# mudit1729/dinov2-od

Hardware: AMD Instinct MI355X
Metric: images/sec forward, DINOv2 ViT-B/14 518x518 + 100-query head (higher is better)
Workload: dtype bf16; 1 GPU; ViT-B/14 518x518 bf16, 100 queries, batch 64 per GPU (BASELINE configs[2]'s batch of 64; it fits one GPU, so every GPU runs the whole configuration: weak scaling); global_batch=64, per_gpu_batch=64, image=518, queries=100, parallelism=dp1, hipgraph=True, n_ranks_seen=1, micro_batches=2

## Files before the change

### dinov2_od_amd/_native.py

```python
import ctypes as C
import os

_HERE = os.path.dirname(os.path.abspath(__file__))
LIB_PATH = os.environ.get("DINODET_LIB") or os.path.join(_HERE, "lib", "libdinodet.so")

DOD_F32, DOD_BF16 = 0, 1
PREC = {"fp32": 0, "bf16": 1, "fp8": 2, "bf16x3": 3, "fp16x2": 4}
ACT = {"none": 0, "relu": 1, "gelu": 2, "sigmoid": 3, "swiglu_pairs": 4}
PW = {"gelu_bwd": 0, "swiglu_bwd": 1, "relu_drop_bwd": 2, "dropout_add": 3, "sigmoid_bwd4": 4}


class DodConfig(C.Structure):
    _fields_ = [
        ("hidden", C.c_int32), ("layers", C.c_int32), ("heads", C.c_int32), ("swiglu", C.c_int32),
        ("patch", C.c_int32), ("pos_grid", C.c_int32), ("ffn_hidden", C.c_int32), ("ln_eps", C.c_float),
        ("lora_r", C.c_int32), ("lora_alpha", C.c_float), ("target_dim", C.c_int32),
        ("num_queries", C.c_int32), ("dec_hidden", C.c_int32), ("dec_heads", C.c_int32),
        ("dec_layers", C.c_int32), ("num_classes", C.c_int32), ("dim_feedforward", C.c_int32),
        ("n_points", C.c_int32), ("use_deformable", C.c_int32), ("dec_ln_eps", C.c_float),
        ("precision", C.c_int32),
    ]


_P, _I, _F, _SZ, _I64 = C.c_void_p, C.c_int, C.c_float, C.c_size_t, C.c_int64


class DodDetection(C.Structure):
    _fields_ = [("image_id", C.c_int64), ("category_id", C.c_int32), ("query", C.c_int32), ("bbox", C.c_float * 4),
                ("score", C.c_float), ("reserved", C.c_int32)]

DEC_TRAIN_FIELDS = ["query_embed", "class_w", "class_b", "bb0_w", "bb0_b", "bb2_w", "bb2_b", "in_proj_w", "in_proj_b", "out_proj_w",
                    "out_proj_b", "norm1_w", "norm1_b", "norm2_w", "norm2_b", "norm3_w", "norm3_b", "lin1_w", "lin1_b", "lin2_w", "lin2_b",
                    "refp_w", "refp_b", "off_w", "off_b", "aw_w", "aw_b", "vp_w", "vp_b", "op_w", "op_b"]


class DodDecTrainParams(C.Structure):
    _fields_ = [(f, C.c_void_p) for f in DEC_TRAIN_FIELDS]


DENSE_LAYER_FIELDS = ["sa_in_w", "sa_in_b", "sa_out_w", "sa_out_b", "ca_in_w", "ca_in_b", "ca_out_w", "ca_out_b", "lin1_w", "lin1_b", "lin2_w", "lin2_b",
                      "norm1_w", "norm1_b", "norm2_w", "norm2_b", "norm3_w", "norm3_b"]


class DodDenseLayerParams(C.Structure):
    _fields_ = [(f, C.c_void_p) for f in DENSE_LAYER_FIELDS]


class DodDenseDecTrainParams(C.Structure):
    _fields_ = [("nlayers", C.c_int32), ("reserved", C.c_int32), ("layers", C.POINTER(DodDenseLayerParams))] + \
               [(f, C.c_void_p) for f in ("query_embed", "class_w", "class_b", "bb0_w", "bb0_b", "bb2_w", "bb2_b")]


class DodLoraLinear(C.Structure):
    _fields_ = [("w", C.c_void_p), ("b", C.c_void_p), ("A", C.c_void_p), ("Bm", C.c_void_p)]


class DodBbBlockParams(C.Structure):
    _fields_ = [(f, C.c_void_p) for f in ("ln1_w", "ln1_b", "ln2_w", "ln2_b", "ls1", "ls2")] + \
               [(f, DodLoraLinear) for f in ("q", "k", "v", "o", "fc1", "fc2")]


class DodBbTailParams(C.Structure):
    _fields_ = [("nblocks", C.c_int32), ("reserved", C.c_int32), ("blocks", C.POINTER(DodBbBlockParams)),
                ("lnf_w", C.c_void_p), ("lnf_b", C.c_void_p), ("proj_w", C.c_void_p), ("proj_b", C.c_void_p)]


class DodOptimTensor(C.Structure):
    _fields_ = [("p", C.c_void_p), ("g", C.c_void_p), ("m", C.c_void_p), ("v", C.c_void_p), ("n", C.c_int64),
                ("step_size", C.c_float), ("bc2_sqrt", C.c_float)]


class DodLnFold(C.Structure):
    _fields_ = [("stats", C.c_void_p), ("csum", C.c_void_p), ("op_out", C.c_void_p), ("part", C.c_void_p), ("shift", C.c_void_p),
                ("part_in", C.c_void_p), ("stats_out", C.c_void_p), ("eps", C.c_float)]


class DodDrawLayer(C.Structure):
    _fields_ = [("boxes", C.c_void_p), ("counts", C.c_void_p), ("labels", C.c_void_p), ("scores", C.c_void_p), ("K", C.c_int32),
                ("format", C.c_int32), ("score_threshold", C.c_float), ("use_palette", C.c_int32), ("color", C.c_uint8 * 4)]


class DodDrawStyle(C.Structure):
    _fields_ = [("thickness", C.c_int32), ("fill_alpha", C.c_int32), ("font_scale", C.c_int32), ("palette_size", C.c_int32),
                ("palette", C.c_void_p), ("names", C.c_void_p), ("n_names", C.c_int32), ("name_len", C.c_int32), ("font", C.c_void_p)]


TUNING_SYMBOLS = {
    "dod_debug_gemm_stamps": (_I, [_P]),
    "dod_debug_pp_stamps": (_I, [_P]),
    "dod_debug_attn_stamps": (_I, [_P]),
    "dod_debug_mfma_peak": (_I, [_I, _I, _I, _P, _P]),
    "dod_debug_mfma_valu_probe": (_I, [_I, _I, _I, _I, _P, _P]),
}

SYMBOLS = {
    "dod_create": (_I, [C.POINTER(DodConfig), C.POINTER(_P)]),
    "dod_destroy": (None, [_P]),
    "dod_last_error": (C.c_char_p, [_P]),
    "dod_set_weight": (_I, [_P, C.c_char_p, _P, C.POINTER(C.c_int64), _I, _I]),
    "dod_finalize_weights": (_I, [_P, _P]),
    "dod_prepare": (_I, [_P, _I, _I, _P]),
    "dod_workspace_bytes": (_SZ, [_P, _I, _I, _I]),
    "dod_num_tokens": (_I, [_P, _I, _I]),
    "dod_forward": (_I, [_P, _P, _I, _I, _I, _P, _P, _SZ, _P]),
    "dod_forward_u8": (_I, [_P, _P, _I, _I, _I, _P, _P, _SZ, _P]),
    "dod_backbone_forward": (_I, [_P, _P, _I, _I, _I, _P, _P, _SZ, _P]),
    "dod_backbone_prefix": (_I, [_P, _P, _I, _I, _I, _I, _P, _P, _SZ, _P]),
    "dod_decoder_forward": (_I, [_P, _P, _I, _I, _P, _P, _SZ, _P]),
    "dod_decoder_workspace_bytes": (_SZ, [_P, _I, _I]),
    "dod_set_tap": (_I, [_P, _I, _P]),
    "dod_profile": (_I, [_P, _I]),
    "dod_profile_read": (_I, [_P, _I, C.POINTER(C.c_double), C.POINTER(C.c_double), C.POINTER(C.c_int)]),
    "dod_op_linear": (_I, [_I, _P, _I, _P, _I, _I, _I, _I, _P, _P, _P, _I, _P, _I, _I, _I, _P]),
    "dod_op_gemm_f32x": (_I, [_P, _I, _I, C.c_longlong, C.c_longlong, _P, _I, _I, C.c_longlong, C.c_longlong, _P, _I, C.c_longlong, C.c_longlong,
                         _I, _I, _I, _I, _I, _F, _I, _I, _P]),
    "dod_op_gemm_f32x3": (_I, [_P, _I, _I, C.c_longlong, C.c_longlong, _P, _I, _I, C.c_longlong, C.c_longlong, _P, _I, C.c_longlong, C.c_longlong,
                          _I, _I, _I, _I, _I, _F, _I, _I, _P]),
    "dod_op_linear_f32x3": (_I, [_P, _I, _P, _P, _P, _P, _I, _I, _I, _I, _P, _I, _I, _P]),
    "dod_op_linear_fp8": (_I, [_P, _I, _P, _P, _I, _P, _I, _I, _I, _P, _P, _P, _I, _P, _I, _I, _I, _P]),
    "dod_op_quant_rows_fp8": (_I, [_P, _I, _I, _I, _I, _P, _I, _P, _P]),
    "dod_op_quant_mx_fp8": (_I, [_P, _I, _I, _I, _I, _P, _I, _P, _P]),
    "dod_op_linear_fp8_glu_mx": (_I, [_P, _I, _P, _P, _I, _P, _I, _I, _I, _P, _P, _I, _P, _P]),
    "dod_op_linear_fp8_mx": (_I, [_P, _I, _P, _P, _I, _P, _I, _I, _I, _P, _P, _P, _I, _P, _I, _I, _I, _P]),
    "dod_op_linear_fp8_mx2": (_I, [_P, _I, _P, _P, _I, _P, _I, _I, _I, _P, _P, _P, _I, _P, _I, _I, _I, _P, _P]),
    "dod_op_split_pair": (_I, [_P, _I, _I, _I, _P, _P]),
    "dod_op_linear_x3": (_I, [_P, _P, _I, _I, _I, _P, _P, _P, _I, _P, _I, _I, _I, _P]),
    "dod_op_attention_x3": (_I, [_P, _P, _I, _I, _I, _F, _P]),
    "dod_op_attention_x3_h2": (_I, [_P, _P, _I, _I, _I, _F, _P]),
    "dod_op_split_h2": (_I, [_P, _I, _I, _I, _P, _P, _P]),
    "dod_op_linear_h2": (_I, [_P, _P, _P, _I, _I, _I, _P, _P, _P, _I, _P, _I, _I, _I, _P]),
    "dod_op_layernorm": (_I, [_P, _P, _P, _P, _F, _I, _I, _P, _I, _P]),
    "dod_op_linear_ln": (_I, [_I, _P, _P, _P, _I, _I, _I, _P, _P, _P, _I, _P, _I, _I, _I, C.POINTER(DodLnFold), _P]),
    "dod_op_rowstats": (_I, [_P, _I, _I, _F, _P, _I, _P, _P]),
    "dod_op_ln_finalize": (_I, [_P, _I, _I, _F, _P, _P]),
    "dod_op_attention_bf16": (_I, [_P, _P, _I, _I, _I, _F, _P]),
    "dod_op_attention_bf16_mx": (_I, [_P, _P, _P, _I, _I, _I, _F, _P]),
    "dod_op_attention_f32": (_I, [_P, _P, _P, _P, _I, _I, _I, _I, _I, _I, _I, _I, _I, _F, _P]),
    "dod_op_deform_sample": (_I, [_P, _I, _P, _I, _I, _I, _I, _I, _I, _I, _I, _P, _P]),
    "dod_op_pos_resize": (_I, [_P, _I, _I, _I, _I, _P, _P]),
    "dod_op_im2col": (_I, [_P, _I, _I, _I, _I, _I, _P, _I, _P]),
    "dod_postprocess_workspace_bytes": (_SZ, [_I, _I, _I]),
    "dod_postprocess": (_I, [_P, _I, _I, _I, _P, _F, _P, C.c_int64, _P, _P, _SZ, _P]),
    "dod_detect_workspace_bytes": (_SZ, [_I, _I, _I, _I]),
    "dod_detect": (_I, [_P, _I, _I, _I, _I, _P, _F, _I, _F, _I, _I, _P, _P, _P, _P, _P, _P, _SZ, _P]),
    "dod_detect_views_workspace_bytes": (_SZ, [_I, _I, _I, _I]),
    "dod_detect_views": (_I, [_P, _I, _I, _I, _I, _P, _P, _P, _P, _I, _F, _I, _F, _I, _I, _I, _F, _P, _P, _P, _P, _P, _P, _P, _SZ, _P]),
    "dod_fuse_views_workspace_bytes": (_SZ, [_I, _I, _I, _I]),
    "dod_fuse_views": (_I, [_P, _I, _I, _I, _I, _P, _P, _P, _P, _I, _F, _I, _F, _I, _I, _F, _I, _P, _P, _P, _P, _P, _P, _P, _P, _SZ, _P]),
    "dod_draw_detections": (_I, [_P, _I, _I, _I, _I, C.POINTER(DodDrawLayer), C.POINTER(DodDrawLayer), C.POINTER(DodDrawStyle), _P, _P]),
    "dod_preprocess": (_I, [_P, _P, _P, _P, _I, _I, _I, _I, _I, _P, _P, _P, _P]),
    "dod_preprocess_u8": (_I, [_P, _P, _P, _P, _I, _I, _I, _I, _I, _P, _P, _P, _P]),
    "dod_preprocess_aug": (_I, [_P, _P, _P, _P, _I, _P, _P, _P, _P, _I, _I, _I, _I, _P, _P, _P, _P]),
    "dod_preprocess_aug_u8": (_I, [_P, _P, _P, _P, _I, _P, _P, _P, _P, _I, _I, _I, _I, _P, _P, _P, _P]),
    "dod_preprocess_compose": (_I, [_P, _P, _P, _P, _I, _P, _P, _I, _I, _P, _P, _P, _I, _I, _I, _I, _I, _I, _P, _P, _P, _P]),
    "dod_preprocess_compose_u8": (_I, [_P, _P, _P, _P, _I, _P, _P, _I, _I, _P, _P, _P, _I, _I, _I, _I, _I, _I, _P, _P, _P, _P]),
    "dod_match_cost": (_I, [_P, _I, _I, _I, _P, _P, _P, _I, _F, _F, _F, _F, _F, _I, _P, _P]),
    "dod_match_assign_workspace_bytes": (_SZ, [_I, _I, _I]),
    "dod_match_assign": (_I, [_P, _P, _I, _I, _I, _P, _I, _P, _P, _P, _SZ, _P]),
    "dod_coco_eval_workspace_bytes": (_SZ, [_I64, _I, _I, _I64]),
    "dod_coco_eval_set_gt": (_I, [_P, _SZ, _I64, _I, _I, _I64, _P, _P, _P, _P, _P, _P, _P, _P, _P]),
    "dod_coco_eval_reset": (_I, [_P, _SZ, _I64, _I, _I, _I64, _P]),
    "dod_coco_eval_append": (_I, [_P, _SZ, _I64, _I, _I, _I64, _P, _P, _I64, _P]),
    "dod_coco_eval_append_host": (_I, [_P, _SZ, _I64, _I, _I, _I64, _P, _I64, _P]),
    "dod_coco_eval_evaluate": (_I, [_P, _SZ, _I64, _I, _I, _I64, _P, _P, _P, _P, _P, _P]),
    "dod_coco_eval_matches": (_I, [_P, _SZ, _I64, _I, _I, _I64, _I64, _P, _P, _P, _P, _I, _P, _P, _P]),
    "dod_op_sort_pairs_workspace_bytes": (_SZ, [_I64]),
    "dod_op_sort_pairs_u64": (_I, [_P, _P, _P, _P, _I64, _I, _I, _P, _SZ, _P]),
    "dod_set_criterion_workspace_bytes": (_SZ, [_I, _I, _I]),
    "dod_set_criterion_forward": (_I, [_P, C.c_int64, _P, C.c_int64, _I, _I, _I, _P, _P, _I, _P, _I, _P, _F, _F, _P, _P, _P, _SZ, _P]),
    "dod_set_criterion_backward": (_I, [_P, C.c_int64, _P, C.c_int64, _I, _I, _I, _P, _P, _I, _P, _I, _P, _F, _F, _P, _P, _P, _P, _P]),
    "dod_set_criterion_layers_workspace_bytes": (_SZ, [_I, _I, _I, _I]),
    "dod_set_criterion_layers_forward": (_I, [_P, C.c_int64, _P, C.c_int64, _I, _I, _I, _I, _P, _P, _I, _P, _I, _P, _F, _F, _P, _P, _P, _SZ, _P]),
    "dod_set_criterion_layers_backward": (_I, [_P, C.c_int64, _P, C.c_int64, _I, _I, _I, _I, _P, _P, _I, _P, _I, _P, _F, _F, _P, _P, _P, _P, _P]),
    "dod_decoder_train_aux_tape_bytes": (_SZ, [C.POINTER(DodConfig), _I, _I]),
    "dod_decoder_train_aux_workspace_bytes": (_SZ, [C.POINTER(DodConfig), _I, _I]),
    "dod_decoder_train_aux_forward": (_I, [C.POINTER(DodConfig), _P, _P, _I, _I, _F, C.c_uint64, _P, _P, _SZ, _P, _SZ, _P]),
    "dod_decoder_train_aux_backward": (_I, [C.POINTER(DodConfig), _P, _P, _I, _I, _F, C.c_uint64, _P, _P, _SZ, _P, _P, _P, _SZ, _P]),
    "dod_decoder_train_tape_bytes": (_SZ, [C.POINTER(DodConfig), _I, _I]),
    "dod_decoder_train_workspace_bytes": (_SZ, [C.POINTER(DodConfig), _I, _I]),
    "dod_decoder_train_forward": (_I, [C.POINTER(DodConfig), _P, _P, _I, _I, _F, C.c_uint64, _P, _P, _SZ, _P, _SZ, _P]),
    "dod_decoder_train_backward": (_I, [C.POINTER(DodConfig), _P, _P, _I, _I, _F, C.c_uint64, _P, _P, _SZ, _P, _P, _P, _SZ, _P]),
    "dod_decoder_train_last_error": (C.c_char_p, []),
    "dod_dense_decoder_train_tape_bytes": (_SZ, [C.POINTER(DodConfig), _I, _I]),
    "dod_dense_decoder_train_workspace_bytes": (_SZ, [C.POINTER(DodConfig), _I, _I]),
    "dod_dense_decoder_train_forward": (_I, [C.POINTER(DodConfig), _P, _P, _I, _I, _F, C.c_uint64, _P, _P, _SZ, _P, _SZ, _P]),
    "dod_dense_decoder_train_backward": (_I, [C.POINTER(DodConfig), _P, _P, _I, _I, _F, C.c_uint64, _P, _P, _SZ, _P, _P, _P, _SZ, _P]),
    "dod_backbone_tail_tape_bytes": (_SZ, [C.POINTER(DodConfig), _I, _I, _I]),
    "dod_backbone_tail_workspace_bytes": (_SZ, [C.POINTER(DodConfig), _I, _I, _I]),
    "dod_backbone_tail_train_forward": (_I, [C.POINTER(DodConfig), _P, _P, _I, _I, _P, _P, _SZ, _P, _SZ, _P]),
    "dod_backbone_tail_train_backward": (_I, [C.POINTER(DodConfig), _P, _I, _I, _P, _P, _SZ, _P, _P, _SZ, _P]),
    "dod_op_layernorm_bwd": (_I, [_P, _P, _P, _F, _I, _I, _P, _P, _P, _P]),
    "dod_op_attention_f32_vjp_workspace_bytes": (_SZ, [_I, _I, _I, _I, _I, _I]),
    "dod_op_attention_f32_vjp": (_I, [_P, _I, _P, _P, _I, _P, _P, _I, _P, _I, _P, _P, _I, _I, _I, _I, _I, _I, _F, _I, _F, C.c_uint64, _P, _SZ, _P]),
    "dod_op_deform_sample_bwd": (_I, [_P, _I, _P, _P, _I, _I, _I, _I, _I, _I, _I, _I, _P, _P, _P]),
    "dod_op_lora_grads_workspace_bytes": (_SZ, [_I, _I]),
    "dod_op_lora_grads": (_I, [_P, _I, _P, _I, _I, _P, _P, _I, _I, _F, _P, _P, _P, _SZ, _P]),
    "dod_op_train_pointwise": (_I, [_I, _P, _P, _P, _SZ, _I, _F, C.c_uint64, _P]),
    "dod_op_colsum_add": (_I, [_P, _I, _I, _I, _P, _P]),
    "dod_optim_workspace_bytes": (_SZ, [_I, _I64]),
    "dod_optim_clip_grad_norm": (_I, [_P, _I, _F, _P, _P, _SZ, _P]),
    "dod_optim_adam_step": (_I, [_P, _I, C.c_double, C.c_double, _F, C.c_double, _F, _P, _P, _SZ, _P]),
    "dod_optim_last_error": (C.c_char_p, []),
    "dod_reserve_gemm_scratch": (_I, [C.c_size_t]),
    "dod_test_set_option": (_I, [C.c_char_p, _I]),
    "dod_test_counter": (C.c_long, [C.c_char_p]),
    "dod_test_gemm_plan": (_I, [_I, _I, _I, _I, C.c_uint, _I, C.c_size_t, _P, _I]),
    "dod_version": (C.c_char_p, []),
    "dod_abi_version": (_I, []),
    "dod_device_count": (_I, []),
}

_lib = None
ABI_VERSION = 6


def lib():
    global _lib
    if _lib is None:
        import torch
        if not os.path.exists(LIB_PATH):
            raise RuntimeError(
                f"{LIB_PATH} not found: the HIP extension is required (no CPU fallback). "
                "Build it with `python -m dinov2_od_amd._build`.")
        L = C.CDLL(LIB_PATH)
        other = bool(os.environ.get("DINODET_LIB"))
        for name, (res, args) in SYMBOLS.items():
            if other and not hasattr(L, name):
                continue
            fn = getattr(L, name)
            fn.restype = res
            fn.argtypes = args
        for name, (res, args) in TUNING_SYMBOLS.items():
            if hasattr(L, name):
                fn = getattr(L, name)
                fn.restype = res
                fn.argtypes = args
        if L.dod_abi_version() != ABI_VERSION and not other:
            raise RuntimeError(f"{LIB_PATH} has ABI revision {L.dod_abi_version()}, this binding expects {ABI_VERSION}: rebuild it "
                               "(`python -m dinov2_od_amd._build --force`)")
        try:
            if torch.cuda.is_available() and L.dod_device_count() <= 0:
                raise RuntimeError("libdinodet.so is bound to a different HIP runtime than PyTorch "
                                   "(it sees no device): import torch before loading it")
        except AttributeError:
            pass
        _lib = L
    return _lib


class DodGemmStep(C.Structure):
    _fields_ = [(n, C.c_int) for n in ("form", "row0", "rows", "kslices", "regmath", "gm")]


def gemm_plan(family, M, N, K, epi_flags, cus, scratch_bytes):
    steps = (DodGemmStep * 4)()
    n = lib().dod_test_gemm_plan(family, M, N, K, epi_flags, cus, scratch_bytes, steps, 4)
    if n < 0:
# ... 30 lines not shown
```

### dinov2_od_amd/csrc/dod_api.hip

```cpp
#include "dod_internal.h"
#include "gemm_plan.h"

#include <cstdarg>
#include <cstdio>
#include <atomic>
#include <cstdlib>

using namespace dod;

static std::string g_err;

static int vfail(const dod_handle* h, int code, const char* fmt, va_list ap, int launch_rc = 0) {
  char buf[512];
  const int n = vsnprintf(buf, sizeof buf, fmt, ap);
  if (launch_rc && n >= 0 && (size_t)n < sizeof buf) snprintf(buf + n, sizeof buf - n, " rejected (rc %d)", launch_rc);
  if (h) h->err = buf; else g_err = buf;
  return code;
}
int dod::fail(const dod_handle* h, int code, const char* fmt, ...) {
  va_list ap; va_start(ap, fmt); code = vfail(h, code, fmt, ap); va_end(ap);
  return code;
}
int dod::rejected(const dod_handle* h, int r, const char* fmt, ...) {
  if (!r) return DOD_OK;
  va_list ap; va_start(ap, fmt); const int code = vfail(h, r == 3 ? DOD_ERR_HIP : DOD_ERR_INVALID, fmt, ap, r); va_end(ap);
  return code;
}

static bool check_common(dod_handle* h, int B, int H, int W, int* rc) {
  if (!h) { *rc = fail(nullptr, DOD_ERR_INVALID, "null handle"); return false; }
  if (!h->finalized) { *rc = fail(h, DOD_ERR_STATE, "dod_finalize_weights has not been called"); return false; }
  if (B <= 0) { *rc = fail(h, DOD_ERR_INVALID, "batch must be positive (got %d)", B); return false; }
  if (H < h->cfg.patch || W < h->cfg.patch) { *rc = fail(h, DOD_ERR_INVALID, "image %dx%d smaller than one %dx%d patch", H, W, h->cfg.patch, h->cfg.patch); return false; }
  return true;
}

static std::atomic<int> g_options[DOD_OPT_COUNT] = {{-1}, {-1}, {-1}, {-1}, {-1}, {-1}, {-1}, {-1}, {-1}, {-1}, {-1}};
int dod_option(int which) { return which >= 0 && which < DOD_OPT_COUNT ? g_options[which].load() : -1; }
static const char* const k_option_names[DOD_OPT_COUNT] = {"tailsplit", "dec_fused_split", "mha_chunk_images", "no_fused_patch", "ln_fold", "deterministic", "f32_ksplit",
                                                       "attn_bwd_flash", "epi_regmath", "f32x3_tile", "attn_diet"};

static std::atomic<long> g_form_launches[FORM_COUNT];
static const char* const k_form_names[FORM_COUNT] = {"bf16_128_r2", "bf16_128_r3", "bf16_m16", "k64", "ppm", "x3_16w", "x3_pp", "h2", "fp8_rows", "fp8mx_256x128",
                                                     "fp8mx2_256x128", "fp8mx2_256x256", "f32", "patch_fused"};
void gemm_form_launched(int form) { if (form >= 0 && form < FORM_COUNT) ++g_form_launches[form]; }

extern "C" {

int dod_test_set_option(const char* name, int value) {
  if (!name) return fail(nullptr, DOD_ERR_INVALID, "null option name");
  for (int i = 0; i < DOD_OPT_COUNT; ++i)
    if (!strcmp(name, k_option_names[i])) { g_options[i].store(value); return DOD_OK; }
  return fail(nullptr, DOD_ERR_INVALID, "unknown test option '%s'", name);
}
long dod_test_counter(const char* name) {
  if (name && !strcmp(name, "tail_splits")) return gemm_tail_split_count();
  if (name && !strcmp(name, "rem_cuts")) return gemm_rem_cut_count();
  if (name && !strcmp(name, "f32_ksplits")) return gemm_f32_ksplit_count();
  if (name && !strcmp(name, "epi_regmath")) return gemm_epi_regmath_count();
  if (name && !strcmp(name, "attn_diet")) return attn_half_tile_count();
  if (name && !strcmp(name, "f32x3_launches")) return gemm_f32x3_count(0);
  if (name && !strcmp(name, "f32x3_wide_launches")) return gemm_f32x3_count(1);
  if (name && !strcmp(name, "optim_launches")) return optim_launch_count();
  if (name && !strcmp(name, "optim_chunk_elems")) return optim_constant(0);
  if (name && !strcmp(name, "optim_table_tensors")) return optim_constant(1);
  if (name && !strcmp(name, "optim_norm_table_tensors")) return optim_constant(2);
  if (name && !strncmp(name, "form_", 5))
    for (int i = 0; i < FORM_COUNT; ++i)
      if (!strcmp(name + 5, k_form_names[i])) return g_form_launches[i].load();
  return -1;
}

int dod_test_gemm_plan(int family, int M, int N, int K, unsigned epi_flags, int cus, size_t scratch_bytes, dod_gemm_step* steps, int max_steps) {
  if (family < GEMM_BF16 || family > GEMM_F32 || M <= 0 || N <= 0 || K <= 0 || cus <= 0 || !steps) return -1;
  const GemmPlan pl = gemm_plan(family, M, N, K, epi_flags, gemm_policy(cus, scratch_bytes, scratch_bytes > 0));
  if (pl.n > 4 || pl.n > max_steps) return -1;
  for (int i = 0; i < pl.n; ++i) {
    const GemmStep& st = pl.step[i];
    steps[i].form = st.form; steps[i].row0 = st.row0; steps[i].rows = st.rows; steps[i].kslices = st.kslices; steps[i].regmath = st.regmath; steps[i].gm = st.gm;
  }
  return pl.n;
}

const char* dod_version(void) { return "dinodet 0.3 (gfx950)"; }
int dod_abi_version(void) { return DOD_ABI_VERSION; }

int dod_device_count(void) {
  int n = 0;
  return hipGetDeviceCount(&n) == hipSuccess ? n : -1;
}

const char* dod_last_error(const dod_handle* h) { return h ? h->err.c_str() : g_err.c_str(); }

int dod_create(const dod_config* cfg, dod_handle** out) {
  if (!cfg || !out) return fail(nullptr, DOD_ERR_INVALID, "null argument");
  const dod_config& c = *cfg;
  if (c.hidden <= 0 || c.layers <= 0 || c.heads <= 0 || c.hidden % c.heads) return fail(nullptr, DOD_ERR_INVALID, "bad backbone dims hidden=%d heads=%d layers=%d", c.hidden, c.heads, c.layers);
  if (c.hidden % 64) return fail(nullptr, DOD_ERR_INVALID, "hidden (%d) must be a multiple of 64", c.hidden);
  {
    const int fm = c.precision == DOD_PREC_FP32 ? 4 : 64;
    if (c.ffn_hidden <= 0 || c.ffn_hidden % fm) return fail(nullptr, DOD_ERR_INVALID, "ffn_hidden (%d) must be a multiple of %d in this precision", c.ffn_hidden, fm);
  }
  if (c.patch <= 0 || c.pos_grid <= 0) return fail(nullptr, DOD_ERR_INVALID, "bad patch/pos_grid");
  if (c.num_queries <= 0 || c.dec_hidden <= 0 || c.dec_heads <= 0 || c.dec_layers <= 0 || c.num_classes <= 0 || c.dim_feedforward <= 0) return fail(nullptr, DOD_ERR_INVALID, "bad decoder dims");
  if (c.dec_hidden % 64 || c.dim_feedforward % 4) return fail(nullptr, DOD_ERR_INVALID, "decoder hidden (%d) must be a multiple of 64, dim_feedforward (%d) of 4", c.dec_hidden, c.dim_feedforward);
  if (c.target_dim && c.target_dim != c.dec_hidden) return fail(nullptr, DOD_ERR_INVALID, "projection dim %d != decoder hidden %d", c.target_dim, c.dec_hidden);
  if (!c.target_dim && c.hidden != c.dec_hidden) return fail(nullptr, DOD_ERR_INVALID, "backbone width %d != decoder hidden %d and no projection", c.hidden, c.dec_hidden);
  if (c.use_deformable && (c.n_points <= 0 || c.n_points > 8)) return fail(nullptr, DOD_ERR_INVALID, "n_points must be 1..8");
  if (c.dec_layers > 64) return fail(nullptr, DOD_ERR_INVALID, "at most 64 decoder layers");
  if (c.precision != DOD_PREC_FP32 && c.precision != DOD_PREC_BF16 && c.precision != DOD_PREC_FP8 && c.precision != DOD_PREC_BF16X3 && c.precision != DOD_PREC_FP16X2) return fail(nullptr, DOD_ERR_INVALID, "unknown precision %d", c.precision);
  dod_handle* h = new (std::nothrow) dod_handle();
  if (!h) return fail(nullptr, DOD_ERR_STATE, "out of host memory");
  h->cfg = c;
  *out = h;
  return DOD_OK;
}

void dod_destroy(dod_handle* h) {
  if (!h) return;
  for (auto& r : h->prof) { (void)hipEventDestroy(r.a); (void)hipEventDestroy(r.b); }
  for (auto e : h->evpool) (void)hipEventDestroy(e);
  for (void* p : h->owned) (void)hipFree(p);
  delete h;
}

int dod_set_weight(dod_handle* h, const char* key, const void* dev_ptr, const int64_t* shape, int ndim, int dtype) {
  if (!h || !key || !dev_ptr || ndim < 0 || ndim > 8 || (ndim && !shape)) return fail(h, DOD_ERR_INVALID, "dod_set_weight: bad argument");
  if (dtype != DOD_F32 && dtype != DOD_BF16) return fail(h, DOD_ERR_INVALID, "dod_set_weight('%s'): dtype %d is neither DOD_F32 nor DOD_BF16", key, dtype);
  std::string k(key);
  if (k.rfind("module.", 0) == 0) k = k.substr(7);
  WRef r; r.raw = dev_ptr; r.dtype = dtype; r.ptr = dtype == DOD_F32 ? (const float*)dev_ptr : nullptr; r.shape.assign(shape, shape + ndim);
  h->w[k] = r;
  h->finalized = false;
  return DOD_OK;
}

int dod_reserve_gemm_scratch(size_t bytes) { return (gemm_tail_reserve(bytes) || gemm_f32_ksplit_reserve()) ? fail(nullptr, DOD_ERR_HIP, "scratch allocation of %zu bytes failed", bytes) : DOD_OK; }

int dod_finalize_weights(dod_handle* h, void* stream) {
  if (!h) return fail(nullptr, DOD_ERR_INVALID, "null handle");
  { static const size_t mb = [] { const char* v = getenv("DINODET_GEMM_SCRATCH_MB"); return v && atoi(v) > 0 ? (size_t)atoi(v) : (size_t)64; }();
    (void)gemm_tail_reserve(mb << 20);
    (void)gemm_f32_ksplit_reserve(); }
  int rc = finalize_impl(h, (hipStream_t)stream);
  if (rc || !h->has_dec) return rc;
  hipStream_t s = (hipStream_t)stream;
  const dod_config& g = h->cfg;
  const size_t Q = g.num_queries, Dd = g.dec_hidden;
  h->l0_tgt = h->l0_proj = nullptr;
  Carver sz(nullptr);
  const size_t bytes = carve_decoder(h, sz, 1, 1, nullptr, false) + 256;
  void* tmp = nullptr;
  float *t0 = nullptr, *p0 = nullptr;
  HIPCHK(h, hipMalloc(&tmp, bytes));
  if (hipMalloc((void**)&t0, Q * Dd * 4) != hipSuccess || (g.use_deformable && hipMalloc((void**)&p0, Q * (size_t)h->ncat * 4) != hipSuccess)) {
    (void)hipFree(tmp); if (t0) (void)hipFree(t0);
    return fail(h, DOD_ERR_HIP, "allocation of the decoder's layer-0 constants failed");
  }
  h->owned.push_back(t0); if (p0) h->owned.push_back(p0);
  Carver cv((void*)(((uintptr_t)tmp + 255) & ~(uintptr_t)255));
  DecWS dw;
  carve_decoder(h, cv, 1, 1, &dw, false);
  rc = decoder_impl(h, nullptr, 1, 1, dw, nullptr, s, true);
  if (!rc) {
    hipError_t e1 = hipMemcpyAsync(t0, dw.tgt, Q * Dd * 4, hipMemcpyDeviceToDevice, s);
    hipError_t e2 = p0 ? hipMemcpyAsync(p0, dw.proj, Q * (size_t)h->ncat * 4, hipMemcpyDeviceToDevice, s) : hipSuccess;
    hipError_t e3 = hipStreamSynchronize(s);
    if (e1 != hipSuccess || e2 != hipSuccess || e3 != hipSuccess) rc = fail(h, DOD_ERR_HIP, "decoder layer-0 constants: %s", hipGetErrorString(e3 != hipSuccess ? e3 : (e1 != hipSuccess ? e1 : e2)));
  } else (void)hipStreamSynchronize(s);
  (void)hipFree(tmp);
  if (rc) return rc;
  h->l0_tgt = t0; h->l0_proj = p0;
  return DOD_OK;
}

int dod_prepare(dod_handle* h, int H, int W, void* stream) {
  if (!h) return fail(nullptr, DOD_ERR_INVALID, "null handle");
  return prepare_impl(h, H, W, (hipStream_t)stream);
}

int dod_num_tokens(const dod_handle* h, int H, int W) { return h ? (H / h->cfg.patch) * (W / h->cfg.patch) + 1 : 0; }

size_t dod_workspace_bytes(const dod_handle* h, int B, int H, int W) {
  if (!h || B <= 0 || H < h->cfg.patch || W < h->cfg.patch) return 0;
  const int N = dod_num_tokens(h, H, W);
  Carver c(nullptr);
  carve_backbone(h, c, B, N, nullptr);
  carve_decoder(h, c, B, N, nullptr, false);
  return c.off + 256;
}

size_t dod_decoder_workspace_bytes(const dod_handle* h, int B, int N) {
  if (!h || B <= 0 || N <= 0) return 0;
  Carver c(nullptr);
  carve_decoder(h, c, B, N, nullptr, true);
  return c.off + 256;
}

int dod_set_tap(dod_handle* h, int stage, float* dst) {
  if (!h) return fail(nullptr, DOD_ERR_INVALID, "null handle");
  if (dst) h->taps[stage] = dst; else h->taps.erase(stage);
  return DOD_OK;
}

int dod_forward(dod_handle* h, const float* pixels, int B, int H, int W, float* det, void* workspace, size_t wsb, void* stream) {
  int rc;
  if (!check_common(h, B, H, W, &rc)) return rc;
  if (!pixels || !det || !workspace) return fail(h, DOD_ERR_INVALID, "null buffer");
  if (wsb < dod_workspace_bytes(h, B, H, W)) return fail(h, DOD_ERR_STATE, "workspace too small: %zu < %zu", wsb, dod_workspace_bytes(h, B, H, W));
  const int N = dod_num_tokens(h, H, W);
  Carver c(align_ws(workspace));
  BbWS bw; DecWS dw;
  carve_backbone(h, c, B, N, &bw);
  carve_decoder(h, c, B, N, &dw, false);
  CARVE_FITS(h, c, workspace, wsb)
  rc = backbone_impl(h, pixels, B, H, W, bw, nullptr, true, (hipStream_t)stream); if (rc) return rc;
  return decoder_impl(h, bw.mem, B, N, dw, det, (hipStream_t)stream);
}

int dod_forward_u8(dod_handle* h, const uint8_t* pixels_hwc, int B, int H, int W, float* det, void* workspace, size_t wsb, void* stream) {
  int rc;
  if (!check_common(h, B, H, W, &rc)) return rc;
  if (!pixels_hwc || !det || !workspace) return fail(h, DOD_ERR_INVALID, "null buffer");
  if (wsb < dod_workspace_bytes(h, B, H, W)) return fail(h, DOD_ERR_STATE, "workspace too small: %zu < %zu", wsb, dod_workspace_bytes(h, B, H, W));
  const int N = dod_num_tokens(h, H, W);
  Carver c(align_ws(workspace));
  BbWS bw; DecWS dw;
  carve_backbone(h, c, B, N, &bw);
  carve_decoder(h, c, B, N, &dw, false);
  CARVE_FITS(h, c, workspace, wsb)
  rc = backbone_impl(h, nullptr, B, H, W, bw, nullptr, true, (hipStream_t)stream, -1, nullptr, pixels_hwc); if (rc) return rc;
  return decoder_impl(h, bw.mem, B, N, dw, det, (hipStream_t)stream);
}

int dod_backbone_forward(dod_handle* h, const float* pixels, int B, int H, int W, float* features, void* workspace, size_t wsb, void* stream) {
  int rc;
  if (!check_common(h, B, H, W, &rc)) return rc;
  if (!pixels || !features || !workspace) return fail(h, DOD_ERR_INVALID, "null buffer");
  if (wsb < dod_workspace_bytes(h, B, H, W)) return fail(h, DOD_ERR_STATE, "workspace too small: %zu < %zu", wsb, dod_workspace_bytes(h, B, H, W));
  const int N = dod_num_tokens(h, H, W);
  Carver c(align_ws(workspace));
  BbWS bw;
  carve_backbone(h, c, B, N, &bw);
  CARVE_FITS(h, c, workspace, wsb)
  return backbone_impl(h, pixels, B, H, W, bw, features, false, (hipStream_t)stream);
}

int dod_backbone_prefix(dod_handle* h, const float* pixels, int B, int H, int W, int nblocks, float* x_out, void* workspace, size_t wsb, void* stream) {
  int rc;
  if (!check_common(h, B, H, W, &rc)) return rc;
  if (!pixels || !x_out || !workspace) return fail(h, DOD_ERR_INVALID, "null buffer");
  if (nblocks < 0 || nblocks > h->cfg.layers) return fail(h, DOD_ERR_INVALID, "nblocks %d outside 0..%d", nblocks, h->cfg.layers);
  if (wsb < dod_workspace_bytes(h, B, H, W)) return fail(h, DOD_ERR_STATE, "workspace too small: %zu < %zu", wsb, dod_workspace_bytes(h, B, H, W));
  const int N = dod_num_tokens(h, H, W);
  Carver c(align_ws(workspace));
  BbWS bw;
  carve_backbone(h, c, B, N, &bw);
  CARVE_FITS(h, c, workspace, wsb)
  return backbone_impl(h, pixels, B, H, W, bw, nullptr, false, (hipStream_t)stream, nblocks, x_out);
}

int dod_decoder_forward(dod_handle* h, const float* memory, int B, int N, float* det, void* workspace, size_t wsb, void* stream) {
  if (!h) return fail(nullptr, DOD_ERR_INVALID, "null handle");
  if (!h->finalized) return fail(h, DOD_ERR_STATE, "dod_finalize_weights has not been called");
  if (B <= 0 || N <= 0) return fail(h, DOD_ERR_INVALID, "bad B=%d N=%d", B, N);
  if (!memory || !det || !workspace) return fail(h, DOD_ERR_INVALID, "null buffer");
  if (wsb < dod_decoder_workspace_bytes(h, B, N)) return fail(h, DOD_ERR_STATE, "workspace too small");
  Carver c(align_ws(workspace));
  DecWS dw;
  carve_decoder(h, c, B, N, &dw, true);
  CARVE_FITS(h, c, workspace, wsb)
  hipStream_t s = (hipStream_t)stream;
  const void* mem_op = memory;
  if (is_bf16(h)) {
    KCHK(h, launch_cast_bf16(memory, (bf16_t*)dw.mem_op, (size_t)B * N * h->cfg.dec_hidden, s));
    mem_op = dw.mem_op;
  }
  return decoder_impl(h, mem_op, B, N, dw, det, s);
}

int dod_profile(dod_handle* h, int enable) {
  if (!h) return fail(nullptr, DOD_ERR_INVALID, "null handle");
  for (auto& r : h->prof) { h->evpool.push_back(r.a); h->evpool.push_back(r.b); }
  h->prof.clear();
  h->prof_on = enable != 0;
  return DOD_OK;
}

int dod_profile_read(dod_handle* h, int cls, double* ms, double* flops, int* launches) {
  if (!h || cls < 0 || cls >= PC_COUNT) return fail(h, DOD_ERR_INVALID, "bad profile class");
  double t = 0, f = 0; int n = 0;
  for (auto& r : h->prof) {
    if (r.cls != cls) continue;
    HIPCHK(h, hipEventSynchronize(r.b));
    float e = 0.f;
    HIPCHK(h, hipEventElapsedTime(&e, r.a, r.b));
    t += e; f += r.flops; ++n;
  }
  if (ms) *ms = t; if (flops) *flops = f; if (launches) *launches = n;
  return DOD_OK;
}

int dod_op_linear(int in_dtype, const void* A, int lda, const void* W, int ldw, int M, int N, int K, const float* bias,
                  const float* scale, const float* resid, int ldr, void* out, int out_dtype, int ldc, int act, void* stream) {
  if (!A || !W || !out) return fail(nullptr, DOD_ERR_INVALID, "null buffer");
  GemmEpi e = epi(bias, out_dtype == DOD_F32 ? (float*)out : nullptr, out_dtype == DOD_BF16 ? out : nullptr, ldc, act, scale, resid, ldr);
  if (act == DOD_ACT_SWIGLU_PAIRS) {
    if (in_dtype != DOD_BF16 || out_dtype != DOD_BF16 || scale || resid || (N & 7)) return fail(nullptr, DOD_ERR_INVALID, "DOD_ACT_SWIGLU_PAIRS: bf16 in / out, N %% 8 == 0, no scale / residual");
    e.act = ACT_NONE; e.glu = 1;
  }
  int r = in_dtype == DOD_BF16 ? launch_gemm_bf16((const bf16_t*)A, lda, (const bf16_t*)W, ldw, M, N, K, e, (hipStream_t)stream)
                               : launch_gemm_f32((const float*)A, lda, (const float*)W, ldw, M, N, K, e, (hipStream_t)stream);
  return rejected(nullptr, r, "dod_op_linear M=%d N=%d K=%d", M, N, K);
}
int dod_op_gemm_f32x(const float* A, int lda, int a_kmajor, long long a_sb, long long a_sh, const float* W, int ldw, int w_kmajor, long long w_sb,
                     long long w_sh, float* C, int ldc, long long c_sb, long long c_sh, int M, int N, int K, int batch, int hb, float alpha,
                     int accumulate, int ksplit, void* stream) {
  if (!A || !W || !C) return fail(nullptr, DOD_ERR_INVALID, "null buffer");
  GemmF32X g; memset(&g, 0, sizeof g);
  g.A = A; g.lda = lda; g.a_kmajor = a_kmajor; g.a_sb = a_sb; g.a_sh = a_sh;
  g.W = W; g.ldw = ldw; g.w_kmajor = w_kmajor; g.w_sb = w_sb; g.w_sh = w_sh;
  g.C = C; g.ldc = ldc; g.c_sb = c_sb; g.c_sh = c_sh;
  g.M = M; g.N = N; g.K = K; g.batch = batch; g.hb = hb; g.alpha = alpha; g.accumulate = accumulate; g.ksplit = ksplit;
  return rejected(nullptr, launch_gemm_f32x(g, (hipStream_t)stream), "dod_op_gemm_f32x M=%d N=%d K=%d batch=%d", M, N, K, batch);
}
int dod_op_gemm_f32x3(const float* A, int lda, int a_kmajor, long long a_sb, long long a_sh, const float* W, int ldw, int w_kmajor, long long w_sb,
                      long long w_sh, float* C, int ldc, long long c_sb, long long c_sh, int M, int N, int K, int batch, int hb, float alpha,
                      int accumulate, int ksplit, void* stream) {
  if (!A || !W || !C) return fail(nullptr, DOD_ERR_INVALID, "null buffer");
  GemmF32X g; memset(&g, 0, sizeof g);
  g.A = A; g.lda = lda; g.a_kmajor = a_kmajor; g.a_sb = a_sb; g.a_sh = a_sh;
  g.W = W; g.ldw = ldw; g.w_kmajor = w_kmajor; g.w_sb = w_sb; g.w_sh = w_sh;
  g.C = C; g.ldc = ldc; g.c_sb = c_sb; g.c_sh = c_sh;
  g.M = M; g.N = N; g.K = K; g.batch = batch; g.hb = hb; g.alpha = alpha; g.accumulate = accumulate; g.ksplit = ksplit;
  return rejected(nullptr, launch_gemm_f32x3(g, (hipStream_t)stream), "dod_op_gemm_f32x3 M=%d N=%d K=%d batch=%d", M, N, K, batch);
}
int dod_op_linear_f32x3(const float* X, int ldx, const float* W, const float* bias, const float* scale, const float* resid, int ldr, int M, int N, int K,
                        float* Y, int ldy, int act, void* stream) {
  if (!X || !W || !Y) return fail(nullptr, DOD_ERR_INVALID, "null buffer");
  if (act < DOD_ACT_NONE || act > DOD_ACT_SIGMOID) return fail(nullptr, DOD_ERR_INVALID, "dod_op_linear_f32x3: activation %d", act);
  GemmF32X g; memset(&g, 0, sizeof g);
  g.A = X; g.lda = ldx; g.W = W; g.ldw = K; g.C = Y; g.ldc = ldy; g.M = M; g.N = N; g.K = K; g.batch = 1; g.hb = 1; g.alpha = 1.0f; g.ksplit = 1;
  g.bias = bias; g.scale = scale; g.resid = resid; g.ldr = ldr; g.act = act;
  return rejected(nullptr, launch_gemm_f32x3(g, (hipStream_t)stream), "dod_op_linear_f32x3 M=%d N=%d K=%d", M, N, K);
}
int dod_op_linear_fp8(const void* A, int lda, const float* a_scale, const void* W, int ldw, const float* w_scale, int M, int N, int K,
                      const float* bias, const float* scale, const float* resid, int ldr, void* out, int out_dtype, int ldc, int act,
                      void* stream) {
  if (!A || !W || !out || !a_scale || !w_scale) return fail(nullptr, DOD_ERR_INVALID, "null buffer");
  GemmEpi e = epi(bias, out_dtype == DOD_F32 ? (float*)out : nullptr, out_dtype == DOD_BF16 ? out : nullptr, ldc, act, scale, resid, ldr);
  e.a_scale = a_scale; e.w_scale = w_scale;
  return rejected(nullptr, launch_gemm_fp8((const unsigned char*)A, lda, (const unsigned char*)W, ldw, M, N, K, e, (hipStream_t)stream), "dod_op_linear_fp8 M=%d N=%d K=%d", M, N, K);
}
int dod_op_linear_fp8_mx(const void* A, int lda, const void* a_block_scales, const void* W, int ldw, const float* w_scale, int M, int N, int K,
                         const float* bias, const float* scale, const float* resid, int ldr, void* out, int out_dtype, int ldc, int act,
                         void* stream) {
  if (!A || !W || !out || !a_block_scales || !w_scale) return fail(nullptr, DOD_ERR_INVALID, "null buffer");
  GemmEpi e = epi(bias, out_dtype == DOD_F32 ? (float*)out : nullptr, out_dtype == DOD_BF16 ? out : nullptr, ldc, act, scale, resid, ldr);
  e.a_bs = (const unsigned char*)a_block_scales; e.w_scale = w_scale;
  return rejected(nullptr, launch_gemm_fp8((const unsigned char*)A, lda, (const unsigned char*)W, ldw, M, N, K, e, (hipStream_t)stream), "dod_op_linear_fp8_mx M=%d N=%d K=%d", M, N, K);
}
int dod_op_linear_fp8_glu_mx(const void* A, int lda, const float* a_scale, const void* W, int ldw, const float* w_scale, int M, int N, int K,
                             const float* bias, void* out_q, int ldq, void* out_block_scales, void* stream) {
  if (!A || !W || !a_scale || !w_scale || !out_q || !out_block_scales) return fail(nullptr, DOD_ERR_INVALID, "null buffer");
  GemmEpi e = epi(bias, nullptr, out_q, ldq);
  e.a_scale = a_scale; e.w_scale = w_scale; e.glu = 1; e.out_bs = (unsigned char*)out_block_scales;
  return rejected(nullptr, launch_gemm_fp8((const unsigned char*)A, lda, (const unsigned char*)W, ldw, M, N, K, e, (hipStream_t)stream), "dod_op_linear_fp8_glu_mx M=%d N=%d K=%d", M, N, K);
}
int dod_op_linear_fp8_mx2(const void* A, int lda, const void* a_block_scales, const void* W, int ldw, const void* w_block_scales, int M, int N, int K,
                          const float* bias, const float* scale, const float* resid, int ldr, void* out, int out_dtype, int ldc, int act,
                          void* glu_out_block_scales, void* stream) {
  if (!A || !W || !out || !a_block_scales || !w_block_scales) return fail(nullptr, DOD_ERR_INVALID, "null buffer");
// ... 125 lines not shown
```

### dinov2_od_amd/csrc/dod_common.h

```cpp
#pragma once
#include <hip/hip_runtime.h>
#include <stdint.h>
#include <stdlib.h>

typedef __attribute__((ext_vector_type(8))) __bf16 bf16x8;
typedef __attribute__((ext_vector_type(4))) __bf16 bf16x4;
typedef __attribute__((ext_vector_type(2))) __bf16 bf16x2;
typedef __attribute__((ext_vector_type(16))) float f32x16;
typedef __attribute__((ext_vector_type(4))) float f32x4;
typedef __attribute__((ext_vector_type(2))) float f32x2;
typedef unsigned short bf16_t;

#define DOD_WAVE 64

enum { DOD_OPT_TAILSPLIT = 0,
       DOD_OPT_DEC_FUSED_SPLIT,
       DOD_OPT_MHA_CHUNK_IMAGES,
       DOD_OPT_NO_FUSED_PATCH,
       DOD_OPT_LN_FOLD,
       DOD_OPT_DETERMINISTIC,
       DOD_OPT_F32_KSPLIT,
       DOD_OPT_ATTN_BWD_FLASH,
       DOD_OPT_EPI_REGMATH,
       DOD_OPT_F32X3_TILE,
       DOD_OPT_ATTN_DIET,
       DOD_OPT_COUNT };
int dod_option(int which);
long gemm_tail_split_count();
long optim_launch_count();
long optim_constant(int which);
long gemm_rem_cut_count();
long attn_half_tile_count();
long gemm_epi_regmath_count();
enum { FORM_BF16_128_R2 = 0, FORM_BF16_128_R3, FORM_BF16_M16, FORM_K64, FORM_PPM, FORM_X3_16W, FORM_X3_PP, FORM_H2, FORM_FP8_ROWS, FORM_FP8MX_256X128,
       FORM_FP8MX2_256X128, FORM_FP8MX2_256X256, FORM_F32, FORM_PATCH_FUSED, FORM_COUNT };
void gemm_form_launched(int form);
enum { GEMM_BF16 = 0, GEMM_X3, GEMM_H2, GEMM_FP8, GEMM_F32 };

#ifdef DINODET_TUNING
#define DOD_TUNE_ENV(name) getenv(name)
#else
#define DOD_TUNE_ENV(name) (static_cast<const char*>(nullptr))
#endif

__device__ __forceinline__ bf16_t f2bf(float f) {
  __bf16 b = (__bf16)f;
  return __builtin_bit_cast(bf16_t, b);
}
__device__ __forceinline__ float bf2f(bf16_t h) {
  return __builtin_bit_cast(float, ((uint32_t)h) << 16);
}
__device__ __forceinline__ uint32_t pack2bf(float lo, float hi) {
  f32x2 v = {lo, hi};
  bf16x2 h = __builtin_convertvector(v, bf16x2);
  return __builtin_bit_cast(uint32_t, h);
}
__device__ __forceinline__ float wave_sum(float v) {
#pragma unroll
  for (int o = 32; o > 0; o >>= 1) v += __shfl_xor(v, o, 64);
  return v;
}
__device__ __forceinline__ float wave_max(float v) {
#pragma unroll
  for (int o = 32; o > 0; o >>= 1) v = fmaxf(v, __shfl_xor(v, o, 64));
  return v;
}
__device__ __forceinline__ unsigned pack4_fp8(float a, float b, float c, float d) {
  int w = __builtin_amdgcn_cvt_pk_fp8_f32(a, b, 0, false);
  w = __builtin_amdgcn_cvt_pk_fp8_f32(c, d, w, true);
  return (unsigned)w;
}
__device__ __forceinline__ unsigned mx_ebyte(float amax) {
  const unsigned b = __float_as_uint(amax * (1.0f / 448.0f));
  unsigned eb = ((b >> 23) & 0xffu) + ((b & 0x7fffffu) ? 1u : 0u);
  eb = eb < 1u ? 1u : (eb > 253u ? 253u : eb);
  return eb;
}
__device__ __forceinline__ float mx_inv_scale(unsigned eb) { return __uint_as_float((254u - eb) << 23); }
__device__ __forceinline__ size_t mx_scale_off(int K, int bi) { return (size_t)(bi & 1) * (K >> 6) + (bi >> 1); }
typedef __attribute__((ext_vector_type(2))) _Float16 f16x2;
typedef __attribute__((ext_vector_type(8))) _Float16 f16x8;
__device__ __forceinline__ float clampf_(float v, float lim) { return __builtin_fminf(__builtin_fmaxf(v, -lim), lim); }
__device__ __forceinline__ void h2_quad(float4 v, float shi, uint2& f16, unsigned& hi8, unsigned& lo8) {
  v.x = clampf_(v.x, 65504.f); v.y = clampf_(v.y, 65504.f); v.z = clampf_(v.z, 65504.f); v.w = clampf_(v.w, 65504.f);
  const f16x2 p0 = {(_Float16)v.x, (_Float16)v.y}, p1 = {(_Float16)v.z, (_Float16)v.w};
  f16.x = __builtin_bit_cast(unsigned, p0); f16.y = __builtin_bit_cast(unsigned, p1);
  const float hx = (float)p0.x, hy = (float)p0.y, hz = (float)p1.x, hw = (float)p1.y;
  const float slo = shi * 2048.0f;
  hi8 = pack4_fp8(clampf_(hx * shi, 448.f), clampf_(hy * shi, 448.f), clampf_(hz * shi, 448.f), clampf_(hw * shi, 448.f));
  lo8 = pack4_fp8(clampf_((v.x - hx) * slo, 448.f), clampf_((v.y - hy) * slo, 448.f), clampf_((v.z - hz) * slo, 448.f), clampf_((v.w - hw) * slo, 448.f));
}
__device__ __forceinline__ size_t h2_off8(int K, int c) { return (size_t)2 * K + (size_t)(c >> 4) * 32 + (c & 15); }

__device__ __forceinline__ float gelu_erf(float x) { return 0.5f * x * (1.0f + erff(x * 0.70710678118654752440f)); }
typedef float f32x2_t __attribute__((ext_vector_type(2)));
__device__ __forceinline__ f32x2_t gelu_fast2(f32x2_t x) {
  f32x2_t ax; ax.x = __builtin_fabsf(x.x); ax.y = __builtin_fabsf(x.y);
  const f32x2_t z = ax * 0.8493218002880191f;
  const f32x2_t d = __builtin_elementwise_fma(z, (f32x2_t)(0.2727374808792225f), (f32x2_t)(1.0f));
  f32x2_t t; t.x = __builtin_amdgcn_rcpf(d.x); t.y = __builtin_amdgcn_rcpf(d.y);
  f32x2_t p = __builtin_elementwise_fma(t, (f32x2_t)(0.5f * 1.061405429f), (f32x2_t)(0.5f * -1.453152027f));
  p = __builtin_elementwise_fma(p, t, (f32x2_t)(0.5f * 1.421413741f));
  p = __builtin_elementwise_fma(p, t, (f32x2_t)(0.5f * -0.284496736f));
  p = __builtin_elementwise_fma(p, t, (f32x2_t)(0.5f * 0.254829592f));
  const f32x2_t nz2 = -z * z;
  f32x2_t e; e.x = __builtin_amdgcn_exp2f(nz2.x); e.y = __builtin_amdgcn_exp2f(nz2.y);
  const f32x2_t q = ax * (t * p);
  const f32x2_t r = __builtin_elementwise_fma(ax, (f32x2_t)(0.5f), x * 0.5f);
  return __builtin_elementwise_fma(-q, e, r);
}
__device__ __forceinline__ void gelu_fast4(float4& v) {
  f32x2_t a = {v.x, v.y}, b = {v.z, v.w};
  a = gelu_fast2(a); b = gelu_fast2(b);
  v.x = a.x; v.y = a.y; v.z = b.x; v.w = b.y;
}
__device__ __forceinline__ float sigmoidf_(float x) { return 1.0f / (1.0f + expf(-x)); }

enum { ACT_NONE = 0, ACT_RELU = 1, ACT_GELU = 2, ACT_SIGMOID = 3 };

struct GemmEpi {
  const float* bias;
  const float* scale;
  const float* resid;
  int ldr;
  float* out_f32;
  bf16_t* out_bf16;
  int ldc;
  int act;
  const float* pos;
  int rows_per_img;
  int out_rows_per_img;
  int out_split;
  const float* a_scale;
  const float* w_scale;
  unsigned char* out_bs;
  const unsigned char* a_bs;
  const unsigned char* w_bs;
  int out_h2;
  const unsigned char* h2_wexp;
  int ksplit;
  int kslice_len;
  long long kslice_stride;
  int glu;
  void* ln_op;
  int ln_op_kind;
  int ln_op_ld;
  float2* ln_part;
  int ln_npart;
  const float2* ln_shift;
  const float2* ln_stats;
  const float* ln_c;
  const float2* ln_part_in;
  float2* ln_stats_out;
  float ln_eps;
};
enum { LNOP_BF16 = 1, LNOP_PAIR = 2, LNOP_H2 = 3 };
inline bool gemm_epi_rows_ok(const GemmEpi& e) {
  return e.rows_per_img == 0 && !e.pos && e.ksplit <= 1 && !e.a_scale && !e.a_bs && !e.out_bs;
}
inline GemmEpi gemm_epi_rows(const GemmEpi& e, int m0) {
  GemmEpi r = e;
  const size_t m = (size_t)m0;
  if (r.resid) r.resid += m * r.ldr;
  if (r.out_f32) r.out_f32 += m * r.ldc;
  if (r.out_bf16) r.out_bf16 += m * r.ldc;
  if (r.ln_op) r.ln_op = reinterpret_cast<char*>(r.ln_op) + m * (size_t)r.ln_op_ld * 2;
  if (r.ln_part) r.ln_part += m * r.ln_npart;
  if (r.ln_shift) r.ln_shift += m;
  if (r.ln_stats) r.ln_stats += m;
  if (r.ln_part_in) r.ln_part_in += m * r.ln_npart;
  if (r.ln_stats_out) r.ln_stats_out += m;
  return r;
}

int launch_gemm_bf16(const bf16_t* A, int lda, const bf16_t* W, int ldw, int M, int N, int K,
                     const GemmEpi& e, hipStream_t s);
int launch_gemm_f32(const float* A, int lda, const float* W, int ldw, int M, int N, int K,
                    const GemmEpi& e, hipStream_t s, bool allow_ksplit = false);
int gemm_f32_ksplit_reserve();
long gemm_f32_ksplit_count();
struct GemmF32X {
  const float* A; const float* W; float* C; const float* bias;
  const float* scale;
  const float* resid;
  int ldr;
  int lda, ldw, ldc, M, N, K;
  long long a_sb, a_sh, w_sb, w_sh, c_sb, c_sh;
  int batch, hb;
  int a_kmajor, w_kmajor;
  float alpha;
  int accumulate;
  int act;
  int ksplit;
};
int launch_gemm_f32x(const GemmF32X& g, hipStream_t s);
int launch_gemm_f32x3(const GemmF32X& g, hipStream_t s);
long gemm_f32x3_count(int wide);
int launch_quant_mx_fp8(const void* x, int in_bf16, int ld, int rows, int cols, unsigned char* q, int ldq, unsigned char* bs, hipStream_t s);
int launch_gemm_fp8(const unsigned char* A, int lda, const unsigned char* W, int ldw, int M, int N, int K,
                    const GemmEpi& e, hipStream_t s);
int launch_attn_x3(const bf16_t* qkv2, bf16_t* ctx3, int B, int N, int heads, float scale, hipStream_t s, int ctx_h2 = 0);
int launch_swiglu_fp8(const bf16_t* in, int rows, int Fh, unsigned char* q, float* scale, hipStream_t s);
int launch_quant_rows_fp8(const void* x, int in_bf16, int ld, int rows, int cols, unsigned char* q, int ldq, float* scale,
                          hipStream_t s);

struct LnOut {
  float* f32 = nullptr;
  bf16_t* bf16 = nullptr;
  unsigned char* fp8 = nullptr;
  float* scale = nullptr;
  bf16_t* split = nullptr;
  bf16_t* a3 = nullptr;
  unsigned char* bs = nullptr;
};
inline LnOut ln_out(float* f32, bf16_t* bf16 = nullptr, bf16_t* a3 = nullptr) { LnOut o; o.f32 = f32; o.bf16 = bf16; o.a3 = a3; return o; }
int launch_layernorm(const float* x, const float* add, const float* gamma, const float* beta, float eps, int rows, int D, const LnOut& out,
                     hipStream_t s, int split_h2 = 0);
int launch_rowstats(const float* x, int rows, int D, float eps, void* op, int op_kind, float2* stats, hipStream_t s);
int launch_ln_finalize(const float2* part, int npart, int rows, int D, float eps, float2* stats, hipStream_t s);
int launch_ln_fold(const float* W, int rows, int cols, const float* gamma, const float* beta, const float* bias_in, float* Wout, float* bias_out, hipStream_t s);
int launch_rowsum(const float* W, int rows, int cols, int round_bf16, float* c, hipStream_t s);

int launch_attn_bf16(const bf16_t* qkv, bf16_t* ctx, int B, int N, int heads, float scale, hipStream_t s, unsigned char* ctx_bs = nullptr);

struct AttnF32 {
  const float *q, *k, *v; float* o;
  int ldq, ldk, ldv, ldo;
  int Lq, Lk;
  int B, heads, dh;
  float scale;
  bf16_t* o3 = nullptr;
  float* lse = nullptr;
};
int launch_attn_f32(const AttnF32& a, hipStream_t s);
struct AttnF32Bwd {
  const float *q, *k, *v, *o, *d_o, *lse;
  float *dq, *dk, *dv, *delta;
  int ldq, ldk, ldv, ldo, lddq, lddk, lddv;
  int Lq, Lk, B, heads, dh;
  float scale;
};
int launch_attn_f32_bwd(const AttnF32Bwd& a, hipStream_t s);

int launch_im2col(const float* img, int B, int H, int W, int patch, int Kp, float* out_f32, bf16_t* out_bf16, hipStream_t s);
int launch_patch_pack(const float* W, int D, int p, bf16_t* out, int x3, hipStream_t s);
int launch_patch_embed(const void* img, int u8, int B, int H, int W, int p, const bf16_t* Wp, int x3, const float* bias, const float* pos,
                       float* out, int D, hipStream_t s);
int launch_cls_row(const float* cls, const float* pos, float* x, int B, int N, int D, hipStream_t s);
int launch_pos_resize(const float* pos_in, int G, int gh, int gw, int D, float* pos_out, hipStream_t s);
int launch_interleave_halves(const float* src, float* dst, int F, int cols, hipStream_t s);
int launch_swiglu(const float* in_f32, const bf16_t* in_bf16, int rows, int Fh, float* out_f32, bf16_t* out_bf16, hipStream_t s);
int launch_cast_bf16(const float* in, bf16_t* out, size_t n, hipStream_t s);
int launch_copy2d(const float* src, int ld_src, float* dst, int ld_dst, int rows, int cols, int cols_pad, hipStream_t s);
int launch_lora_merge(const float* W, const float* A, const float* Bm, float alpha, int out_f, int in_f, int r, float* dst, hipStream_t s);
int launch_split3(const float* in, int ld_in, bf16_t* out, int rows, int K, int mode, hipStream_t s);
int launch_split2(const float* in, int ld_in, bf16_t* out, int rows, int K, hipStream_t s);
int launch_split_h2(const float* in, int ld_in, void* out, int rows, int K, unsigned char* wexp, hipStream_t s);
int launch_gemm_h2(const void* A, int lda, const void* W, int ldw, int M, int N, int K, const GemmEpi& e, hipStream_t s);
int launch_gemm_x3(const bf16_t* A2, int lda, const bf16_t* W2, int ldw, int M, int N, int K, const GemmEpi& e, hipStream_t s);
int gemm_dispatch(int family, const void* A, int lda, const void* W, int ldw, int M, int N, int K, const GemmEpi& e, hipStream_t s, bool allow_ksplit = false);
int device_cus();
struct KernelLds { const void* fn; int bytes; };
void gemm_lds_attr_once(bool* done, const KernelLds* k, int n);
int gemm_tile_mode();
int run_gemm_bf16_128(const bf16_t* A, int lda, const bf16_t* W, int ldw, int M, int N, int K, const GemmEpi& e, int slots, hipStream_t s);
int run_gemm_bf16_m16(const bf16_t* A, int lda, const bf16_t* W, int ldw, int M, int N, int K, const GemmEpi& e, int gm, hipStream_t s);
int run_gemm_x3_16w(const bf16_t* A2, int lda, const bf16_t* W2, int ldw, int M, int N, int K, const GemmEpi& e, hipStream_t s);
int run_gemm_k64(const bf16_t* A, int lda, const bf16_t* W, int ldw, int M, int N, int K, const GemmEpi& e, bool regmath, hipStream_t s);
int run_gemm_pp(bool x3, const bf16_t* A, int lda, const bf16_t* W, int ldw, int M, int N, int K, const GemmEpi& e, hipStream_t s);
int run_gemm_h2(const void* A, int lda, const void* W, int ldw, int M, int N, int K, const GemmEpi& e, hipStream_t s);
int run_gemm_ksplit_reduce(const float* part, int S, int R, int N, const GemmEpi& e, int m_base, int M, int K, hipStream_t s);
int run_gemm_fp8(int form, const unsigned char* A, int lda, const unsigned char* W, int ldw, int M, int N, int K, const GemmEpi& e, int gm, hipStream_t s);
int run_gemm_f32(const float* A, int lda, const float* W, int ldw, int M, int N, int K, const GemmEpi& e, int S, hipStream_t s);
int gemm_tail_reserve(size_t bytes);
size_t gemm_tail_reserved();
float* gemm_tail_slab(hipStream_t s);
bool gemm_f32_ksplit_reserved();
int launch_bcast_rows(const float* src, float* dst, int B, int rows, int D, hipStream_t s);

int launch_deform_sample(const float* proj, int ldp, const float* values, int B, int Q, int N, int Hd, int P, int dh,
                         int h, int w, float* out, hipStream_t s, int proj_shared = 0, bf16_t* out3 = nullptr);
```

### dinov2_od_amd/csrc/dod_forward.hip

```cpp
#include "dod_internal.h"

#include <cmath>
#include <cstdlib>

using namespace dod;

size_t dod::carve_decoder(const dod_handle* h, Carver& c, int B, int N, DecWS* w, bool need_mem_op) {
  const dod_config& g = h->cfg;
  const size_t BQ = (size_t)B * g.num_queries, Dd = g.dec_hidden, M = (size_t)B * N;
  DecWS t;
  t.tgt = (float*)c.take(BQ * Dd * 4); t.t2 = (float*)c.take(BQ * Dd * 4); t.att = (float*)c.take(BQ * Dd * 4);
  t.samp = (float*)c.take(BQ * Dd * 4); t.qkv = (float*)c.take(BQ * 3 * Dd * 4);
  t.proj = (float*)c.take(BQ * (size_t)(h->ncat > 0 ? h->ncat : 4) * 4);
  t.ffn = (float*)c.take(BQ * (size_t)g.dim_feedforward * 4); t.hb = (float*)c.take(BQ * (Dd / 2) * 4);
  t.qd = (float*)c.take(BQ * Dd * 4);
  { const size_t kmax = Dd > (size_t)g.dim_feedforward ? Dd : (size_t)g.dim_feedforward;
    const bool want3 = is_bf16(h) || is_x3(h);
    t.a3 = want3 ? (bf16_t*)c.take(BQ * 3 * kmax * 2) : nullptr;
    t.a3b = want3 ? (bf16_t*)c.take(BQ * 3 * kmax * 2) : nullptr; }
  t.mem2 = is_x3(h) ? (bf16_t*)c.take(M * 2 * Dd * 2) : nullptr;
  t.mem_op = need_mem_op ? c.take(M * Dd * esz(h)) : nullptr;
  if (g.use_deformable) {
    int uniq = 0; for (auto& L : h->DL) if (L.vp_alias < 0) ++uniq;
    if (!h->finalized) uniq = g.dec_layers;
    t.values = (float*)c.take(M * Dd * 4 * (size_t)(uniq > 0 ? uniq : 1)); t.kv = nullptr;
  } else {
    t.values = nullptr; t.kv = (float*)c.take(M * 2 * Dd * 4);
  }
  if (w) *w = t;
  return c.off;
}

size_t dod::carve_backbone(const dod_handle* h, Carver& c, int B, int N, BbWS* w) {
  const dod_config& g = h->cfg;
  const size_t M = (size_t)B * N, D = g.hidden, es = esz(h), Np = N - 1;
  const size_t F1 = g.swiglu ? 2 * (size_t)g.ffn_hidden : (size_t)g.ffn_hidden;
  size_t hb = M * F1; const size_t col = (size_t)B * Np * (size_t)(h->Kp ? h->Kp : (3 * g.patch * g.patch + 63) / 64 * 64);
  if (col > hb) hb = col;
  BbWS t;
  t.x = (float*)c.take(M * D * 4); t.y = c.take(M * D * es); t.qkv = c.take(M * 3 * D * es); t.ctx = c.take(M * D * es);
  t.hbuf = c.take(hb * es); t.gated = g.swiglu ? c.take(M * (size_t)g.ffn_hidden * es) : nullptr;
  t.mem = c.take(M * (size_t)(g.target_dim ? g.target_dim : g.hidden) * es);
  t.rs = is_fp8(h) ? (float*)c.take(M * 4) : nullptr;
  t.bs = (is_fp8(h) && g.swiglu && g.ffn_hidden % 256 == 0) ? (unsigned char*)c.take(M * (size_t)(g.ffn_hidden / 32)) : nullptr;
  t.bsx = (is_fp8(h) && D % 256 == 0) ? (unsigned char*)c.take(M * (D / 32)) : nullptr;
  const bool foldable = ln_foldable(h);
  t.lnp = foldable ? (float2*)c.take(M * ((D + 127) / 128) * 8) : nullptr;
  t.lns = foldable ? (float2*)c.take(M * 8) : nullptr;
  t.lns2 = foldable ? (float2*)c.take(M * 8) : nullptr;
  if (w) *w = t;
  return c.off;
}

int dod::prepare_impl(dod_handle* h, int H, int W, hipStream_t s) {
  const dod_config& g = h->cfg;
  if (!h->finalized || !h->has_bb) return fail(h, DOD_ERR_STATE, "backbone weights not finalized");
  if (H < g.patch || W < g.patch) return fail(h, DOD_ERR_INVALID, "image %dx%d smaller than one patch", H, W);
  if (h->pos_H == H && h->pos_W == W) return DOD_OK;
  const int gh = H / g.patch, gw = W / g.patch;
  if (gh * gw == g.pos_grid * g.pos_grid && H == W) { h->pos_hw = h->pos; h->pos_H = H; h->pos_W = W; return DOD_OK; }
  const std::pair<int, int> key(gh, gw);
  auto it = h->pos_cache.find(key);
  if (it == h->pos_cache.end()) {
    hipStreamCaptureStatus cs = hipStreamCaptureStatusNone;
    if (s && hipStreamIsCapturing(s, &cs) == hipSuccess && cs != hipStreamCaptureStatusNone)
      return fail(h, DOD_ERR_STATE, "first forward at %dx%d inside a stream capture: call dod_prepare(h, %d, %d) before capturing", H, W, H, W);
    const size_t need = (size_t)(gh * gw + 1) * g.hidden;
    float* buf = nullptr;
    HIPCHK(h, hipMalloc((void**)&buf, need * 4));
    h->owned.push_back(buf);
    KCHK(h, launch_pos_resize(h->pos, g.pos_grid, gh, gw, g.hidden, buf, s));
    it = h->pos_cache.emplace(key, buf).first;
  }
  h->pos_hw = it->second; h->pos_H = H; h->pos_W = W;
  return DOD_OK;
}

namespace {

void spatial_factor(int hw, int* h, int* w) {
  int s = (int)std::sqrt((double)hw);
  while ((s + 1) * (s + 1) <= hw) ++s;
  while (s * s > hw) --s;
  if (s * s != hw) {
    for (int i = s; i > 0; --i) if (hw % i == 0) { *h = i; *w = hw / i; return; }
  }
  *h = s; *w = s;
}

int tap(dod_handle* h, int stage, const void* src, bool src_bf16, size_t n, hipStream_t s) {
  auto it = h->taps.find(stage);
  if (it == h->taps.end() || !it->second) return 0;
  if (!src_bf16) { (void)hipMemcpyAsync(it->second, src, n * 4, hipMemcpyDeviceToDevice, s); return 0; }
  return launch_widen_bf16((const bf16_t*)src, it->second, n, s);
}

int linear(dod_handle* h, bool bf, const void* A, int lda, const void* W, int ldw, int M, int N, int K, const GemmEpi& e, hipStream_t s, int flops_K = 0) {
  ProfScope ps(h, s, bf ? PC_GEMM_BF16 : PC_GEMM_F32, 2.0 * M * N * (e.rows_per_img > 0 ? 3.0 * h->cfg.patch * h->cfg.patch : (double)(flops_K ? flops_K : K)));
  int r = bf ? launch_gemm_bf16((const bf16_t*)A, lda, (const bf16_t*)W, ldw, M, N, K, e, s)
             : launch_gemm_f32((const float*)A, lda, (const float*)W, ldw, M, N, K, e, s, h->cfg.precision != DOD_PREC_FP32);
  return rejected(h, r, "linear launch (M=%d N=%d K=%d bf16=%d)", M, N, K, (int)bf);
}
int linear3(dod_handle* h, const void* A3, const void* W3, int M, int N, int K, const GemmEpi& e, hipStream_t s) {
  ProfScope ps(h, s, PC_GEMM_BF16, 2.0 * M * N * (double)K);
  int r = launch_gemm_x3((const bf16_t*)A3, 2 * K, (const bf16_t*)W3, 2 * K, M, N, K, e, s);
  return rejected(h, r, "bf16x3 linear launch (M=%d N=%d K=%d)", M, N, K);
}

struct Operand {
  const void* rows;
  const float* row_scale = nullptr;
  const unsigned char* bs = nullptr;
};

int block_linear(dod_handle* h, const Operand& a, const PackedLinear& W, int M, int N, int K, GemmEpi e, hipStream_t s) {
  if (is_h2(h)) {
    ProfScope ps(h, s, PC_GEMM_BF16, 2.0 * M * N * (double)K);
    e.h2_wexp = W.wexp;
    return rejected(h, launch_gemm_h2(a.rows, 4 * K, W.W, 3 * K, M, N, K, e, s), "fp16x2 linear launch (M=%d N=%d K=%d)", M, N, K);
  }
  if (is_x3(h)) return linear3(h, a.rows, W.W, M, N, K, e, s);
  if (W.wscale || W.wbs) {
    ProfScope ps(h, s, PC_GEMM_FP8, 2.0 * M * N * (double)K);
    e.a_scale = a.row_scale; e.w_scale = W.wscale; e.a_bs = a.bs; e.w_bs = W.wbs;
    return rejected(h, launch_gemm_fp8((const unsigned char*)a.rows, K, (const unsigned char*)W.W, K, M, N, K, e, s), "fp8 linear launch (M=%d N=%d K=%d)", M, N, K);
  }
  return linear(h, is_bf16(h), a.rows, K, W.W, K, M, N, K, e, s);
}

struct BlockRun {
  dod_handle* h; const BbWS& ws; hipStream_t s;
  int B, N, M, D, F;
  bool bf, f8, x3, h2, fold;
  float scale;
  float2* stat[2];
  int cur = 0;
  bool fresh = false;
  int op_kind, npart;

  BlockRun(dod_handle* h_, const BbWS& ws_, hipStream_t s_, int B_, int N_, bool fold_)
      : h(h_), ws(ws_), s(s_), B(B_), N(N_), M(B_ * N_), D(h_->cfg.hidden), F(h_->cfg.ffn_hidden), bf(is_bf16(h_)), f8(is_fp8(h_)), x3(is_x3(h_)),
        h2(is_h2(h_)), fold(fold_), scale(1.0f / std::sqrt((float)(h_->cfg.hidden / h_->cfg.heads))), stat{ws_.lns, ws_.lns2},
        op_kind(is_h2(h_) ? LNOP_H2 : (is_x3(h_) ? LNOP_PAIR : LNOP_BF16)), npart((h_->cfg.hidden + 127) / 128) {}

  bool mx(const BLayer& L) const { return f8 && L.qkv.wbs && ws.bsx; }

  GemmEpi residual_epi(const PackedLinear& W, const float* layer_scale, bool next_norm_reads) {
    GemmEpi e = epi(W.bias, ws.x, nullptr, D, ACT_NONE, layer_scale, ws.x, D);
    if (fold && next_norm_reads) {
      e.ln_op = ws.y; e.ln_op_kind = op_kind; e.ln_op_ld = (op_kind == LNOP_BF16 ? D : 2 * D); e.ln_part = ws.lnp; e.ln_npart = npart; e.ln_shift = stat[cur];
      fresh = true;
    }
    return e;
  }
  GemmEpi normed_epi(GemmEpi e, const PackedLinear& W) {
    if (fold) {
      e.ln_stats = stat[cur]; e.ln_c = W.csum;
      if (fresh) { e.ln_part_in = ws.lnp; e.ln_npart = npart; e.ln_stats_out = stat[cur ^ 1]; e.ln_eps = h->cfg.ln_eps; cur ^= 1; fresh = false; }
    }
    return e;
  }
  int norm(const BLayer& L, const float* gamma, const float* beta, Operand* y) {
    *y = Operand{ws.y, f8 && !mx(L) ? ws.rs : nullptr, mx(L) ? ws.bsx : nullptr};
    if (fold) return 0;
    LnOut o;
    if (x3) o.split = (bf16_t*)ws.y;
    else if (f8) { o.fp8 = (unsigned char*)ws.y; o.scale = (float*)y->row_scale; o.bs = (unsigned char*)y->bs; }
    else if (bf) o.bf16 = (bf16_t*)ws.y;
    else o.f32 = (float*)ws.y;
    ProfScope ps(h, s, PC_LAYERNORM, 0);
    KCHK(h, launch_layernorm(ws.x, nullptr, gamma, beta, h->cfg.ln_eps, M, D, o, s, h2 ? 1 : 0));
    return 0;
  }
  int attention(const BLayer& L, const Operand& y, Operand* ctx) {
    const int heads = h->cfg.heads;
    const bool flash = D / heads == 64;
    GemmEpi eq = epi(L.qkv.bias, bf ? nullptr : (float*)ws.qkv, bf ? ws.qkv : nullptr, 3 * D);
    if (x3 && flash) { eq = epi(L.qkv.bias, nullptr, ws.qkv, 6 * D); eq.out_split = -3 * D; }
    int rc = block_linear(h, y, L.qkv, M, 3 * D, D, normed_epi(eq, L.qkv), s); if (rc) return rc;
    const double flops = 4.0 * B * (double)N * N * D;
    *ctx = Operand{ws.ctx};
    if (x3 && flash) {
      ProfScope ps(h, s, PC_ATTN_BF16, flops);
      KCHK(h, launch_attn_x3((const bf16_t*)ws.qkv, (bf16_t*)ws.ctx, B, N, heads, scale, s, h2 ? 1 : 0));
    } else if (bf && mx(L)) {
      ProfScope ps(h, s, PC_ATTN_BF16, flops);
      KCHK(h, launch_attn_bf16((const bf16_t*)ws.qkv, (bf16_t*)ws.y, B, N, heads, scale, s, ws.bsx));
      *ctx = Operand{ws.y, nullptr, ws.bsx};
    } else if (bf) {
      { ProfScope ps(h, s, PC_ATTN_BF16, flops); KCHK(h, launch_attn_bf16((const bf16_t*)ws.qkv, (bf16_t*)ws.ctx, B, N, heads, scale, s)); }
      if (f8) {
        KCHK(h, launch_quant_rows_fp8(ws.ctx, 1, D, M, D, (unsigned char*)ws.y, D, ws.rs, s));
        *ctx = Operand{ws.y, ws.rs};
      }
    } else {
      float* o = x3 ? (float*)ws.hbuf : (float*)ws.ctx;
      {
        ProfScope ps(h, s, PC_ATTN_F32, flops);
        AttnF32 a; const float* q = (const float*)ws.qkv;
        a.q = q; a.k = q + D; a.v = q + 2 * D; a.o = o; a.ldq = a.ldk = a.ldv = 3 * D; a.ldo = D;
        a.Lq = a.Lk = N; a.B = B; a.heads = heads; a.dh = D / heads; a.scale = scale;
        KCHK(h, launch_attn_f32(a, s));
      }
      if (x3) KCHK(h, split(o, D, ws.ctx));
    }
    return 0;
  }
  int split(const float* src, int cols, void* dst) {
    return h2 ? launch_split_h2(src, cols, dst, M, cols, nullptr, s) : launch_split2(src, cols, (bf16_t*)dst, M, cols, s);
  }
  int mlp_in(const BLayer& L, const Operand& y, Operand* hidden) {
    const dod_config& g = h->cfg;
    static const bool mx_gate_env = [] { const char* v = DOD_TUNE_ENV("DINODET_FP8_MX_GATE"); return !(v && v[0] == '0'); }();
    const PackedLinear& W = L.fc1;
    int rc;
    if (!g.swiglu) {
      GemmEpi e1 = epi(W.bias, bf ? nullptr : (float*)ws.hbuf, bf ? ws.hbuf : nullptr, F, ACT_GELU);
      if (x3) { e1 = epi(W.bias, nullptr, ws.hbuf, 2 * F, ACT_GELU); if (h2) e1.out_h2 = 1; else e1.out_split = -F; }
      *hidden = Operand{ws.hbuf};
      return block_linear(h, y, W, M, F, D, normed_epi(e1, W), s);
    }
    if (L.glu) {
      GemmEpi eg = epi(W.bias, nullptr, ws.gated, F);
      *hidden = Operand{ws.gated};
      const bool gate_mx = f8 && ws.bs && (mx(L) || (mx_gate_env && F % 256 == 0));
      if (x3) { eg = epi(W.bias, nullptr, ws.hbuf, 2 * F); if (h2) eg.out_h2 = 1; else eg.out_split = -F; *hidden = Operand{ws.hbuf}; }
      else if (gate_mx) { eg.out_bs = ws.bs; *hidden = Operand{ws.gated, nullptr, ws.bs}; }
      else if (f8) eg = epi(W.bias, nullptr, ws.hbuf, F);
      eg.glu = 1;
      rc = block_linear(h, y, W, M, 2 * F, D, normed_epi(eg, W), s); if (rc) return rc;
      if (f8 && !gate_mx) {
        KCHK(h, launch_quant_rows_fp8(ws.hbuf, 1, F, M, F, (unsigned char*)ws.gated, F, ws.rs, s));
        *hidden = Operand{ws.gated, ws.rs};
      }
      return 0;
    }
    rc = block_linear(h, y, W, M, 2 * F, D, normed_epi(epi(W.bias, bf ? nullptr : (float*)ws.hbuf, bf ? ws.hbuf : nullptr, 2 * F), W), s); if (rc) return rc;
    *hidden = Operand{ws.gated};
    if (f8) { KCHK(h, launch_swiglu_fp8((const bf16_t*)ws.hbuf, M, F, (unsigned char*)ws.gated, ws.rs, s)); *hidden = Operand{ws.gated, ws.rs}; }
    else KCHK(h, launch_swiglu(bf ? nullptr : (const float*)ws.hbuf, bf ? (const bf16_t*)ws.hbuf : nullptr, M, F, bf ? nullptr : (float*)ws.gated, bf ? (bf16_t*)ws.gated : nullptr, s));
    if (x3) { KCHK(h, split((const float*)ws.gated, F, ws.hbuf)); *hidden = Operand{ws.hbuf}; }
    return 0;
  }
  int block(const BLayer& L, bool more) {
    if (mx(L) && h->cfg.swiglu && !(L.glu && ws.bs)) return fail(h, DOD_ERR_STATE, "fp8 SwiGLU MLP needs the fused gate (block-scaled rows)");
    Operand y, ctx, hidden;
    int rc = norm(L, L.ln1w, L.ln1b, &y); if (rc) return rc;
    rc = attention(L, y, &ctx); if (rc) return rc;
    rc = block_linear(h, ctx, L.o, M, D, D, residual_epi(L.o, L.ls1, true), s); if (rc) return rc;
    rc = norm(L, L.ln2w, L.ln2b, &y); if (rc) return rc;
    rc = mlp_in(L, y, &hidden); if (rc) return rc;
    return block_linear(h, hidden, L.fc2, M, D, F, residual_epi(L.fc2, L.ls2, more), s);
  }
};

}

int dod::backbone_impl(dod_handle* h, const float* pixels, int B, int H, int W, const BbWS& ws, float* feat_f32, bool want_mem, hipStream_t s,
                       int stop_blocks, float* x_out, const unsigned char* pixels_u8) {
  const dod_config& g = h->cfg;
  const bool bf = is_bf16(h);
  const int D = g.hidden, p = g.patch;
  const int gh = H / p, gw = W / p, Np = gh * gw, N = Np + 1, M = B * N;
  if (!h->has_bb) return fail(h, DOD_ERR_STATE, "no backbone weights were registered");
  if (bf && D / g.heads != 64) return fail(h, DOD_ERR_INVALID, "bf16 attention kernel needs head_dim 64 (got %d)", D / g.heads);
  int rc = prepare_impl(h, H, W, s); if (rc) return rc;
  if (pixels_u8 && !h->Wpe) return fail(h, DOD_ERR_INVALID, "uint8 input needs the fused patch embed (bf16 / bf16x3 / fp8 precision, patch size 14 or 16)");
  if (h->Wpe && (pixels_u8 || W % 2 == 0)) {
    ProfScope ps(h, s, PC_GEMM_BF16, 2.0 * B * Np * (double)D * 3.0 * p * p);
    KCHK(h, launch_patch_embed(pixels_u8 ? (const void*)pixels_u8 : (const void*)pixels, pixels_u8 ? 1 : 0, B, H, W, p, h->Wpe, is_x3(h) ? 1 : 0,
                               h->bpatch, h->pos_hw, ws.x, D, s));
  } else if (is_x3(h) && h->Wpatch2 && (size_t)3 * D * 6 >= (size_t)h->Kp2 * 4) {
    const int K2 = h->Kp2;
    KCHK(h, launch_im2col(pixels, B, H, W, p, K2, (float*)ws.hbuf, nullptr, s));
    KCHK(h, launch_split2((const float*)ws.hbuf, K2, (bf16_t*)ws.qkv, B * Np, K2, s));
    GemmEpi e = epi(h->bpatch, ws.x, nullptr, D);
    e.pos = h->pos_hw; e.rows_per_img = Np; e.out_rows_per_img = N;
    ProfScope ps(h, s, PC_GEMM_BF16, 2.0 * B * Np * (double)D * 3.0 * p * p);
    KCHK(h, launch_gemm_x3((const bf16_t*)ws.qkv, 2 * K2, h->Wpatch2, 2 * K2, B * Np, D, K2, e, s));
  } else {
    KCHK(h, launch_im2col(pixels, B, H, W, p, h->Kp, bf ? nullptr : (float*)ws.hbuf, bf ? (bf16_t*)ws.hbuf : nullptr, s));
    GemmEpi e = epi(h->bpatch, ws.x, nullptr, D);
    e.pos = h->pos_hw; e.rows_per_img = Np; e.out_rows_per_img = N;
    rc = linear(h, bf, ws.hbuf, h->Kp, h->Wpatch, h->Kp, B * Np, D, h->Kp, e, s); if (rc) return rc;
  }
  KCHK(h, launch_cls_row(h->cls, h->pos_hw, ws.x, B, N, D, s));
  tap(h, 0, ws.x, false, (size_t)M * D, s);
  float* yf = bf ? nullptr : (float*)ws.y; bf16_t* yb = bf ? (bf16_t*)ws.y : nullptr;
  const bool x3 = is_x3(h);
  const int nblocks = stop_blocks >= 0 ? (stop_blocks < g.layers ? stop_blocks : g.layers) : g.layers;
  const bool fold = ln_foldable(h) && !h->L.empty() && h->L[0].fold;
  if (fold && !(ws.lnp && ws.lns && ws.lns2)) return fail(h, DOD_ERR_STATE, "internal: the weights were packed with the LayerNorm folded but the workspace has no statistics buffers");
  BlockRun run(h, ws, s, B, N, fold);
  if (fold && nblocks > 0) { ProfScope ps(h, s, PC_LAYERNORM, 0); KCHK(h, launch_rowstats(ws.x, M, D, g.ln_eps, ws.y, run.op_kind, run.stat[0], s)); }
  for (int i = 0; i < nblocks; ++i) {
    rc = run.block(h->L[i], i + 1 < g.layers); if (rc) return rc;
    tap(h, 1 + i, ws.x, false, (size_t)M * D, s);
  }
  if (stop_blocks >= 0) {
    HIPCHK(h, hipMemcpyAsync(x_out, ws.x, (size_t)M * D * 4, hipMemcpyDeviceToDevice, s));
    return DOD_OK;
  }
  if (!g.target_dim) {
    float* of = feat_f32 ? feat_f32 : (bf ? nullptr : (want_mem ? (float*)ws.mem : nullptr));
    bf16_t* ob = (bf && want_mem) ? (bf16_t*)ws.mem : nullptr;
    KCHK(h, launch_layernorm(ws.x, nullptr, h->lnfw, h->lnfb, g.ln_eps, M, D, ln_out(of, ob), s));
    if (!bf && want_mem && feat_f32) HIPCHK(h, hipMemcpyAsync(ws.mem, feat_f32, (size_t)M * D * 4, hipMemcpyDeviceToDevice, s));
  } else {
    const int Dd = g.target_dim;
    if (x3) {
      { LnOut o; o.split = (bf16_t*)ws.y; KCHK(h, launch_layernorm(ws.x, nullptr, h->lnfw, h->lnfb, g.ln_eps, M, D, o, s)); }
      float* dst = feat_f32 ? feat_f32 : (float*)ws.mem;
      rc = linear3(h, ws.y, h->Wproj, M, Dd, D, epi(h->bproj, dst, nullptr, Dd), s); if (rc) return rc;
      if (feat_f32 && want_mem) HIPCHK(h, hipMemcpyAsync(ws.mem, feat_f32, (size_t)M * Dd * 4, hipMemcpyDeviceToDevice, s));
      return DOD_OK;
    }
    KCHK(h, launch_layernorm(ws.x, nullptr, h->lnfw, h->lnfb, g.ln_eps, M, D, ln_out(yf, yb), s));
    if (feat_f32) { rc = linear(h, bf, ws.y, D, h->Wproj, D, M, Dd, D, epi(h->bproj, feat_f32, nullptr, Dd), s); if (rc) return rc; }
    if (want_mem) { rc = linear(h, bf, ws.y, D, h->Wproj, D, M, Dd, D, epi(h->bproj, bf ? nullptr : (float*)ws.mem, bf ? ws.mem : nullptr, Dd), s); if (rc) return rc; }
  }
  return DOD_OK;
}

int dod::decoder_impl(dod_handle* h, const void* mem_op, int B, int N, const DecWS& ws, float* det, hipStream_t s, bool l0_only) {
  const dod_config& g = h->cfg;
  const bool bf = is_bf16(h);
  const int Dd = g.dec_hidden, Q = g.num_queries, Hd = g.dec_heads, Pn = g.n_points, Fd = g.dim_feedforward, C = g.num_classes;
  const int BQ = B * Q, M = B * N, dh = Dd / Hd;
  if (!h->has_dec) return fail(h, DOD_ERR_STATE, "no decoder weights were registered");
  if (Dd % Hd) return fail(h, DOD_ERR_INVALID, "decoder hidden %d not divisible by heads %d", Dd, Hd);
  if (dh > 128 || dh % 4) return fail(h, DOD_ERR_INVALID, "decoder head_dim %d unsupported (<=128, multiple of 4)", dh);
  int rc;
  if (!l0_only) tap(h, 1000, mem_op, bf, (size_t)M * Dd, s);
  const bool x3 = is_x3(h) && ws.mem2;
  if (x3 && !l0_only) KCHK(h, launch_split2((const float*)mem_op, Dd, ws.mem2, M, Dd, s));
  const bool l0_const = !l0_only && h->l0_tgt && (!g.use_deformable || h->l0_proj);
  if (!l0_const) KCHK(h, launch_bcast_rows(h->query, ws.tgt, 1, Q, Dd, s));
  int fh = 0, fw = 0;
  if (g.use_deformable && !l0_only) {
    spatial_factor(N, &fh, &fw);
    int u = 0;
    for (int j = 0; j < g.dec_layers; ++j) {
      DLayer& L = h->DL[j];
      if (L.vp_alias >= 0) continue;
      float* dst = ws.values + (size_t)u * M * Dd; ++u;
      if (x3 && L.vp_w2) rc = linear3(h, ws.mem2, L.vp_w2, M, Dd, Dd, epi(L.vp_b, dst, nullptr, Dd), s);
      else rc = linear(h, bf, mem_op, Dd, L.vp_w, Dd, M, Dd, Dd, epi(L.vp_b, dst, nullptr, Dd), s);
      if (rc) return rc;
    }
    tap(h, 2000, ws.values, false, (size_t)M * Dd, s);
  }
  const float sscale = 1.0f / std::sqrt((float)dh);
  static const int qrows = DOD_TUNE_ENV("DINODET_QSPLIT_ROWS") ? atoi(DOD_TUNE_ENV("DINODET_QSPLIT_ROWS")) : 1024;
  const bool fuse3 = dod_option(DOD_OPT_DEC_FUSED_SPLIT) != 0;
  auto splits = [&](const bf16_t* W3, int rows, int Nout, int ldc, int act) {
    return (bf || x3) && W3 && ws.a3 && rows >= qrows && Nout >= 128 && Nout % 4 == 0 && ldc % 4 == 0 && act != ACT_SIGMOID;
  };
  auto qlinear = [&](const float* A, int K, const float* Wf, const bf16_t* W3, int rows, int Nout, const GemmEpi& e, const bf16_t* A3 = nullptr) -> int {
    if (splits(W3, rows, Nout, e.ldc, e.act)) {
      if (!A3) { KCHK(h, launch_split3(A, K, ws.a3, rows, K, 0, s)); A3 = ws.a3; }
      return linear(h, true, A3, 3 * K, W3, 3 * K, rows, Nout, 3 * K, e, s, K);
    }
    return linear(h, false, A, K, Wf, K, rows, Nout, K, e, s);
  };
  const bf16_t* tgt3 = nullptr;
  auto post_norm = [&](const float* gamma, const float* beta, int rows, bool next_splits) -> int {
    KCHK(h, launch_layernorm(ws.t2, nullptr, gamma, beta, g.dec_ln_eps, rows, Dd, ln_out(ws.tgt, nullptr, next_splits ? ws.a3 : nullptr), s));
    tgt3 = next_splits ? ws.a3 : nullptr;
    return 0;
  };
  auto self_attn = [&](const DLayer& L, int nb) -> int {
    const int rows = nb * Q;
    int r = qlinear(ws.tgt, Dd, L.in_w, L.in_w3, rows, 3 * Dd, epi(L.in_b, ws.qkv, nullptr, 3 * Dd), tgt3); if (r) return r;
    tgt3 = nullptr;
    AttnF32 a; a.q = ws.qkv; a.k = ws.qkv + Dd; a.v = ws.qkv + 2 * Dd; a.o = ws.att; a.ldq = a.ldk = a.ldv = 3 * Dd; a.ldo = Dd;
    a.Lq = a.Lk = Q; a.B = nb; a.heads = Hd; a.dh = dh; a.scale = sscale;
    const bool o3 = fuse3 && splits(L.out_w3, rows, Dd, Dd, ACT_NONE);
    if (o3) a.o3 = ws.a3;
    KCHK(h, launch_attn_f32(a, s));
    r = qlinear(ws.att, Dd, L.out_w, L.out_w3, rows, Dd, epi(L.out_b, ws.t2, nullptr, Dd, ACT_NONE, nullptr, ws.tgt, Dd), o3 ? ws.a3 : nullptr); if (r) return r;
    const bool n3 = fuse3 && !g.use_deformable && nb == B && splits(L.ca_q_w3, rows, Dd, Dd, ACT_NONE);
    return post_norm(L.n1w, L.n1b, rows, n3);
  };
  auto ffn = [&](const DLayer& L, bool last_layer, const bf16_t* L_next_in_w3) -> int {
    const bool f3 = fuse3 && splits(L.l1w3, BQ, Fd, Fd, ACT_RELU) && splits(L.l2w3, BQ, Dd, Dd, ACT_NONE) && Fd % 4 == 0;
    int r;
    if (f3) {
      GemmEpi e1 = epi(L.l1b, nullptr, nullptr, 3 * Fd, ACT_RELU);
      e1.out_bf16 = ws.a3b; e1.out_split = Fd;
      r = qlinear(ws.tgt, Dd, L.l1w, L.l1w3, BQ, Fd, e1, tgt3);
    } else r = qlinear(ws.tgt, Dd, L.l1w, L.l1w3, BQ, Fd, epi(L.l1b, ws.ffn, nullptr, Fd, ACT_RELU), tgt3);
    if (r) return r;
    tgt3 = nullptr;
    r = qlinear(ws.ffn, Fd, L.l2w, L.l2w3, BQ, Dd, epi(L.l2b, ws.t2, nullptr, Dd, ACT_NONE, nullptr, ws.tgt, Dd), f3 ? ws.a3b : nullptr); if (r) return r;
    const bool n3 = fuse3 && (last_layer ? splits(h->bb0_w3, BQ, Dd / 2, Dd / 2, ACT_RELU) : splits(L_next_in_w3, BQ, 3 * Dd, 3 * Dd, ACT_NONE));
    return post_norm(L.n3w, L.n3b, BQ, n3);
  };
  int uniq_idx[64]; { int u = 0; for (int j = 0; j < g.dec_layers && j < 64; ++j) uniq_idx[j] = h->DL[j].vp_alias < 0 ? u++ : -1; }
  for (int j = 0; j < g.dec_layers; ++j) {
    const DLayer& L = h->DL[j];
    const bool const0 = j == 0 && l0_const;
    const bool shared0 = (j == 0 && (B > 1 || const0));
    if (const0) { KCHK(h, launch_bcast_rows(h->l0_tgt, ws.tgt, B, Q, Dd, s)); tgt3 = nullptr; }
    else { rc = self_attn(L, shared0 ? 1 : B); if (rc) return rc; }
    if (g.use_deformable) {
      if (!const0) { rc = linear(h, false, ws.tgt, Dd, L.cat_w, Dd, shared0 ? Q : BQ, h->ncat, Dd, epi(L.cat_b, ws.proj, nullptr, h->ncat), s); if (rc) return rc; }
      if (l0_only) return DOD_OK;
      if (shared0 && !const0) KCHK(h, launch_bcast_rows(ws.tgt, ws.tgt + (size_t)Q * Dd, B - 1, Q, Dd, s));
      const int src = L.vp_alias >= 0 ? L.vp_alias : j;
      const float* vals = ws.values + (size_t)uniq_idx[src] * M * Dd;
      const bool s3 = fuse3 && splits(L.op_w3, BQ, Dd, Dd, ACT_NONE);
      KCHK(h, launch_deform_sample(const0 ? h->l0_proj : ws.proj, h->ncat, vals, B, Q, N, Hd, Pn, dh, fh, fw, ws.samp, s, shared0 ? 1 : 0, s3 ? ws.a3 : nullptr));
      rc = qlinear(ws.samp, Dd, L.op_w, L.op_w3, BQ, Dd, epi(L.op_b, ws.t2, nullptr, Dd, ACT_NONE, nullptr, ws.tgt, Dd), s3 ? ws.a3 : nullptr); if (rc) return rc;
      const bool n3 = fuse3 && splits(L.l1w3, BQ, Fd, Fd, ACT_RELU);
      rc = post_norm(L.n2w, L.n2b, BQ, n3); if (rc) return rc;
    } else {
      if (l0_only) return DOD_OK;
      if (shared0 && !const0) KCHK(h, launch_bcast_rows(ws.tgt, ws.tgt + (size_t)Q * Dd, B - 1, Q, Dd, s));
      rc = qlinear(ws.tgt, Dd, L.ca_q_w, L.ca_q_w3, BQ, Dd, epi(L.ca_q_b, ws.qd, nullptr, Dd), tgt3); if (rc) return rc;
      tgt3 = nullptr;
      if (x3 && L.ca_kv_w2) rc = linear3(h, ws.mem2, L.ca_kv_w2, M, 2 * Dd, Dd, epi(L.ca_kv_b, ws.kv, nullptr, 2 * Dd), s);
      else rc = linear(h, bf, mem_op, Dd, L.ca_kv_w, Dd, M, 2 * Dd, Dd, epi(L.ca_kv_b, ws.kv, nullptr, 2 * Dd), s);
      if (rc) return rc;
      AttnF32 a; a.q = ws.qd; a.k = ws.kv; a.v = ws.kv + Dd; a.o = ws.att; a.ldq = Dd; a.ldk = a.ldv = 2 * Dd; a.ldo = Dd;
      a.Lq = Q; a.Lk = N; a.B = B; a.heads = Hd; a.dh = dh; a.scale = sscale;
      const bool o3 = fuse3 && splits(L.ca_out_w3, BQ, Dd, Dd, ACT_NONE);
      if (o3) a.o3 = ws.a3;
      KCHK(h, launch_attn_f32(a, s));
      rc = qlinear(ws.att, Dd, L.ca_out_w, L.ca_out_w3, BQ, Dd, epi(L.ca_out_b, ws.t2, nullptr, Dd, ACT_NONE, nullptr, ws.tgt, Dd), o3 ? ws.a3 : nullptr); if (rc) return rc;
      const bool n3 = fuse3 && splits(L.l1w3, BQ, Fd, Fd, ACT_RELU);
      rc = post_norm(L.n2w, L.n2b, BQ, n3); if (rc) return rc;
    }
    rc = ffn(L, j + 1 == g.dec_layers, j + 1 < g.dec_layers ? h->DL[j + 1].in_w3 : nullptr); if (rc) return rc;
    tap(h, 3000 + j, ws.tgt, false, (size_t)BQ * Dd, s);
  }
  rc = linear(h, false, ws.tgt, Dd, h->cls_w, Dd, BQ, C, Dd, epi(h->cls_b, det, nullptr, C + 4), s); if (rc) return rc;
  rc = qlinear(ws.tgt, Dd, h->bb0_w, h->bb0_w3, BQ, Dd / 2, epi(h->bb0_b, ws.hb, nullptr, Dd / 2, ACT_RELU), tgt3); if (rc) return rc;
  rc = linear(h, false, ws.hb, Dd / 2, h->bb2_w, Dd / 2, BQ, 4, Dd / 2, epi(h->bb2_b, det + C, nullptr, C + 4, ACT_SIGMOID), s); if (rc) return rc;
  return DOD_OK;
}
```

### dinov2_od_amd/csrc/dod_internal.h

```cpp
#pragma once
#include "dod_common.h"
#include "../../include/dinodet.h"

#include <cstring>
#include <map>
#include <string>
#include <vector>

struct WRef { const float* ptr; std::vector<int64_t> shape; const void* raw = nullptr; int dtype = DOD_F32; size_t numel() const { size_t n = 1; for (auto s : shape) n *= (size_t)s; return n; } };

struct PackedLinear {
  void* W = nullptr;
  float* bias = nullptr;
  const unsigned char* wexp = nullptr;
  const float* wscale = nullptr;
  const unsigned char* wbs = nullptr;
  const float* csum = nullptr;
};
struct BLayer {
  PackedLinear qkv, o, fc1, fc2;
  float *ln1w = nullptr, *ln1b = nullptr, *ln2w = nullptr, *ln2b = nullptr, *ls1 = nullptr, *ls2 = nullptr;
  bool glu = false;
  bool fold = false;
};
struct DLayer {
  float *in_w = nullptr, *in_b = nullptr, *out_w = nullptr, *out_b = nullptr;
  float *n1w = nullptr, *n1b = nullptr, *n2w = nullptr, *n2b = nullptr, *n3w = nullptr, *n3b = nullptr;
  float *l1w = nullptr, *l1b = nullptr, *l2w = nullptr, *l2b = nullptr;
  bf16_t *in_w3 = nullptr, *out_w3 = nullptr, *l1w3 = nullptr, *l2w3 = nullptr, *op_w3 = nullptr, *ca_q_w3 = nullptr, *ca_out_w3 = nullptr;
  float *cat_w = nullptr, *cat_b = nullptr, *op_w = nullptr, *op_b = nullptr, *vp_b = nullptr;
  void* vp_w = nullptr;
  bf16_t* vp_w2 = nullptr;
  bf16_t* ca_kv_w2 = nullptr;
  int vp_alias = -1;
  float *ca_q_w = nullptr, *ca_q_b = nullptr, *ca_kv_b = nullptr, *ca_out_w = nullptr, *ca_out_b = nullptr;
  void* ca_kv_w = nullptr;
};

struct dod_handle {
  dod_config cfg;
  std::map<std::string, WRef> w;
  mutable std::string err;
  bool finalized = false;
  bool has_bb = false, has_dec = false;
  std::vector<void*> owned;
  std::vector<BLayer> L;
  void* Wpatch = nullptr; int Kp = 0;
  bf16_t* Wpatch2 = nullptr; int Kp2 = 0;
  bf16_t* Wpe = nullptr;
  float *bpatch = nullptr, *cls = nullptr, *pos = nullptr, *lnfw = nullptr, *lnfb = nullptr, *bproj = nullptr;
  void* Wproj = nullptr;
  std::vector<DLayer> DL;
  bf16_t* bb0_w3 = nullptr;
  float *query = nullptr, *cls_w = nullptr, *cls_b = nullptr, *bb0_w = nullptr, *bb0_b = nullptr, *bb2_w = nullptr, *bb2_b = nullptr;
  int ncat = 0;
  float *l0_tgt = nullptr, *l0_proj = nullptr;
  std::map<std::pair<int, int>, float*> pos_cache;
  int pos_H = -1, pos_W = -1; float* pos_hw = nullptr;
  std::map<int, float*> taps;
  bool prof_on = false;
  struct ProfRec { hipEvent_t a, b; int cls; double flops; };
  std::vector<ProfRec> prof;
  std::vector<hipEvent_t> evpool;
};

namespace dod {

int fail(const dod_handle* h, int code, const char* fmt, ...) __attribute__((format(printf, 3, 4)));
int rejected(const dod_handle* h, int r, const char* fmt, ...) __attribute__((format(printf, 3, 4)));
#define HIPCHK(h, x) do { hipError_t e_ = (x); if (e_ != hipSuccess) return dod::fail(h, DOD_ERR_HIP, "%s: %s", #x, hipGetErrorString(e_)); } while (0)
#define KCHK(h, x) do { int r_ = (x); if (r_) return dod::rejected(h, r_, "%s", #x); } while (0)

enum { PC_GEMM_BF16 = 0, PC_ATTN_BF16 = 1, PC_GEMM_F32 = 2, PC_ATTN_F32 = 3, PC_LAYERNORM = 4, PC_OTHER = 5, PC_GEMM_FP8 = 6, PC_COUNT = 7 };
struct ProfScope {
  dod_handle* h; hipStream_t s; int cls; double flops; hipEvent_t a = nullptr;
  ProfScope(dod_handle* h_, hipStream_t s_, int cls_, double flops_) : h(h_), s(s_), cls(cls_), flops(flops_) {
    if (!h->prof_on) return;
    a = take();
    if (a) (void)hipEventRecord(a, s);
  }
  hipEvent_t take() {
    hipEvent_t e = nullptr;
    if (!h->evpool.empty()) { e = h->evpool.back(); h->evpool.pop_back(); return e; }
    if (hipEventCreate(&e) != hipSuccess) return nullptr;
    return e;
  }
  ~ProfScope() {
    if (!h->prof_on || !a) return;
    hipEvent_t b = take();
    if (!b) { h->evpool.push_back(a); return; }
    (void)hipEventRecord(b, s);
    h->prof.push_back({a, b, cls, flops});
  }
};

inline bool is_fp8(const dod_handle* h) { return h->cfg.precision == DOD_PREC_FP8; }
inline bool is_x3(const dod_handle* h) { return h->cfg.precision == DOD_PREC_BF16X3 || h->cfg.precision == DOD_PREC_FP16X2; }
inline bool is_h2(const dod_handle* h) { return h->cfg.precision == DOD_PREC_FP16X2; }
inline bool is_bf16(const dod_handle* h) { return h->cfg.precision == DOD_PREC_BF16 || is_fp8(h); }
inline size_t esz(const dod_handle* h) { return is_x3(h) ? 6 : (is_bf16(h) ? 2 : 4); }
inline size_t align_up(size_t x, size_t a = 256) { return (x + a - 1) / a * a; }
inline bool ln_foldable(const dod_handle* h) { return !is_fp8(h) && (is_bf16(h) || is_x3(h)) && h->cfg.hidden % 32 == 0; }

inline GemmEpi epi(const float* bias, float* of32, void* obf, int ldc, int act = ACT_NONE, const float* scale = nullptr, const float* resid = nullptr, int ldr = 0) {
  GemmEpi e; memset(&e, 0, sizeof e);
  e.bias = bias; e.out_f32 = of32; e.out_bf16 = (bf16_t*)obf; e.ldc = ldc; e.act = act; e.scale = scale; e.resid = resid; e.ldr = ldr;
  return e;
}

struct Carver {
  char* base; size_t off = 0;
  explicit Carver(void* b) : base((char*)b) {}
  void* take(size_t bytes) { void* p = base ? base + off : nullptr; off += align_up(bytes); return p; }
};
inline void* align_ws(void* p) { return (void*)(((uintptr_t)p + 255) & ~(uintptr_t)255); }
#define CARVE_FITS(h, c, workspace, wsb)                                                                                      \
  if ((size_t)((c).base - (char*)(workspace)) + (c).off > (wsb))                                                              \
    return dod::fail(h, DOD_ERR_STATE, "internal: workspace carve %zu exceeds the %zu bytes provided", (size_t)((c).base - (char*)(workspace)) + (c).off, (size_t)(wsb));
struct DecWS { float *tgt, *t2, *att, *samp, *qkv, *proj, *ffn, *hb, *qd; void* mem_op; float* values; float* kv; bf16_t* a3; bf16_t* a3b; bf16_t* mem2; };
struct BbWS { float* x; void *y, *qkv, *ctx, *hbuf, *gated, *mem; float* rs; unsigned char* bs; unsigned char* bsx; float2 *lnp, *lns, *lns2; };
size_t carve_decoder(const dod_handle* h, Carver& c, int B, int N, DecWS* w, bool need_mem_op);
size_t carve_backbone(const dod_handle* h, Carver& c, int B, int N, BbWS* w);

int finalize_impl(dod_handle* h, hipStream_t s);
int launch_widen_bf16(const bf16_t* in, float* out, size_t n, hipStream_t s);
int prepare_impl(dod_handle* h, int H, int W, hipStream_t s);
int backbone_impl(dod_handle* h, const float* pixels, int B, int H, int W, const BbWS& ws, float* feat_f32, bool want_mem, hipStream_t s,
                  int stop_blocks = -1, float* x_out = nullptr, const unsigned char* pixels_u8 = nullptr);
int decoder_impl(dod_handle* h, const void* mem_op, int B, int N, const DecWS& ws, float* det, hipStream_t s, bool l0_only = false);

}
```

### dinov2_od_amd/csrc/gemm_f32.hip

```cpp
#include "dod_common.h"
#include "gemm_f32x_epi.h"
#include "gemm_plan.h"
#include <cstdlib>
#include <cstring>
#include <mutex>

#define FBM 64
#define FBN 64
#define FBK 16
#define FLD 66
#define FPD 4

namespace {

template <bool KM, bool VEC>
struct TileLoad {
  const float* base; int ld, rows, kend, r0; int a, b;
  __device__ __forceinline__ void init(const float* base_, int ld_, int rows_, int kend_, int r0_, int tid) {
    base = base_; ld = ld_; rows = rows_; kend = kend_; r0 = r0_;
    if (KM) { a = tid >> 4; b = (tid & 15) * 4; } else { a = tid >> 2; b = (tid & 3) * 4; }
  }
  __device__ __forceinline__ float4 load(int k0) const {
    const int o = KM ? k0 + a : r0 + a, c = KM ? r0 + b : k0 + b;
    const int on = KM ? kend : rows, cn = KM ? rows : kend;
// ... 34 lines not shown
#pragma unroll
  for (int p = 0; p < FPD; ++p) { ra[p] = la.load((kt0 + p) * FBK); rw[p] = lw.load((kt0 + p) * FBK); }
  la.store(sA[0], ra[0], kt0 * FBK);
  lw.store(sW[0], rw[0], kt0 * FBK);
  __syncthreads();
  auto mma = [&](int st) {
    const float* a = &sA[st][wm * 32 + lr];
    const float* w = &sW[st][wn * 32 + lr];
#pragma unroll
    for (int s = 0; s < FBK / 2; ++s) {
      const float av = a[(2 * s + lh) * FLD];
      const float wv = w[(2 * s + lh) * FLD];
      acc = __builtin_amdgcn_mfma_f32_32x32x2f32(wv, av, acc, 0, 0, 0);
    }
  };
  int kt = 0;
  for (; kt + FPD <= nk; kt += FPD) {
#pragma unroll
    for (int j = 0; j < FPD; ++j) {
      ra[j] = la.load((kt0 + kt + j + FPD) * FBK);
      rw[j] = lw.load((kt0 + kt + j + FPD) * FBK);
      mma(j & 1);
      la.store(sA[(j + 1) & 1], ra[(j + 1) % FPD], (kt0 + kt + j + 1) * FBK);
      lw.store(sW[(j + 1) & 1], rw[(j + 1) % FPD], (kt0 + kt + j + 1) * FBK);
      __syncthreads();
    }
  }
#pragma unroll
  for (int j = 0; j < FPD - 1; ++j) {
    if (kt + j < nk) {
      mma(j & 1);
      if (kt + j + 1 < nk) {
        la.store(sA[(j + 1) & 1], ra[j + 1], (kt0 + kt + j + 1) * FBK);
        lw.store(sW[(j + 1) & 1], rw[j + 1], (kt0 + kt + j + 1) * FBK);
      }
      __syncthreads();
    }
  }
}

inline bool vec_ok(const void* p, long long ld, long long s1 = 0, long long s2 = 0) {
  return ((uintptr_t)p & 15) == 0 && ld >= 4 && ld % 4 == 0 && s1 % 4 == 0 && s2 % 4 == 0;
}

}

template <bool VEC>
__global__ __launch_bounds__(256) void gemm_f32_kernel(const float* __restrict__ A, int lda,
                                                       const float* __restrict__ W, int ldw,
                                                       int M, int N, int K, GemmEpi e, float* __restrict__ part, unsigned* __restrict__ counters) {
  __shared__ __attribute__((aligned(16))) float f32_smem[4 * FBK * FLD];
  __shared__ unsigned s_last;
  const int tid = threadIdx.x, lane = tid & 63, wid = tid >> 6;
  const int wm = wid >> 1, wn = wid & 1;
  const int tiles_m = (M + FBM - 1) / FBM;
  const int tn = blockIdx.x / tiles_m, tm = blockIdx.x - tn * tiles_m;
  const int m0 = tm * FBM, n0 = tn * FBN;
  TileLoad<false, VEC> la, lw;
  la.init(A, lda, M, K, m0, tid);
  lw.init(W, ldw, N, K, n0, tid);
  f32x16 acc;
#pragma unroll
  for (int r = 0; r < 16; ++r) acc[r] = 0.f;
  const int S = gridDim.y, nk = (K + FBK - 1) / FBK;
  const int kt0 = (int)((long long)blockIdx.y * nk / S), kt1 = (int)((long long)(blockIdx.y + 1) * nk / S);
  f32_mainloop(la, lw, kt0, kt1, reinterpret_cast<float (*)[FBK * FLD]>(f32_smem),
               reinterpret_cast<float (*)[FBK * FLD]>(f32_smem + 2 * FBK * FLD), acc);
  if (S > 1) {
    const size_t tiles = gridDim.x;
    float* mine = part + ((size_t)blockIdx.y * tiles + blockIdx.x) * (16 * 256) + tid;
#pragma unroll
    for (int r = 0; r < 16; ++r) __hip_atomic_store(mine + r * 256, acc[r], __ATOMIC_RELAXED, __HIP_MEMORY_SCOPE_AGENT);
    asm volatile("s_waitcnt vmcnt(0)" ::: "memory");
    __syncthreads();
    if (tid == 0) {
      const unsigned old = __hip_atomic_fetch_add(&counters[blockIdx.x], 1u, __ATOMIC_RELAXED, __HIP_MEMORY_SCOPE_AGENT);
      s_last = old == (unsigned)(S - 1);
      if (old == (unsigned)(S - 1)) __hip_atomic_store(&counters[blockIdx.x], 0u, __ATOMIC_RELAXED, __HIP_MEMORY_SCOPE_AGENT);
    }
    __syncthreads();
    if (!s_last) return;
#pragma unroll
    for (int r = 0; r < 16; ++r) acc[r] = 0.f;
    for (int sl = 0; sl < S; ++sl) {
      const float* p = part + ((size_t)sl * tiles + blockIdx.x) * (16 * 256) + tid;
#pragma unroll
      for (int r = 0; r < 16; ++r) acc[r] += __hip_atomic_load(p + r * 256, __ATOMIC_RELAXED, __HIP_MEMORY_SCOPE_AGENT);
    }
  }

  const int lr = lane & 31, lh = lane >> 5;
  const int m = m0 + wm * 32 + lr;
  if (m >= M) return;
  size_t orow = (size_t)m;
  const float* posrow = nullptr;
  if (e.rows_per_img > 0) {
    const int b = m / e.rows_per_img, p = m - b * e.rows_per_img;
    orow = (size_t)b * e.out_rows_per_img + 1 + p;
    posrow = e.pos + (size_t)(1 + p) * N;
  }
#pragma unroll
  for (int g = 0; g < 4; ++g) {
#pragma unroll
    for (int t = 0; t < 4; ++t) {
      const int n = n0 + wn * 32 + 8 * g + 4 * lh + t;
      if (n >= N) continue;
      float v = acc[4 * g + t];
      if (e.bias) v += e.bias[n];
      if (e.act == ACT_GELU) v = gelu_erf(v);
      else if (e.act == ACT_RELU) v = fmaxf(v, 0.f);
      else if (e.act == ACT_SIGMOID) v = sigmoidf_(v);
      if (e.scale) v *= e.scale[n];
      if (posrow) v += posrow[n];
      if (e.resid) v += e.resid[orow * e.ldr + n];
      if (e.out_f32) e.out_f32[orow * e.ldc + n] = v;
      else e.out_bf16[orow * e.ldc + n] = f2bf(v);
    }
  }
}

#define F32K_SLOTS 4
static std::mutex g_f32k_mu;
static char* g_f32k[16] = {};
static hipStream_t g_f32k_owner[16][F32K_SLOTS] = {};
static unsigned long long g_f32k_used[16][F32K_SLOTS] = {};
static unsigned long long g_f32k_clock = 0;
static constexpr size_t F32K_SLAB = (size_t)F32K_TILES * 4 + (size_t)F32K_PARTS * 16 * 256 * 4;
int gemm_f32_ksplit_reserve() {
  int dev = 0;
  if (hipGetDevice(&dev) != hipSuccess || dev < 0 || dev >= 16) return 3;
  std::lock_guard<std::mutex> lk(g_f32k_mu);
  if (g_f32k[dev]) return 0;
  char* blk = nullptr;
  if (hipMalloc((void**)&blk, F32K_SLAB * F32K_SLOTS) != hipSuccess) return 3;
  if (hipMemset(blk, 0, F32K_SLAB * F32K_SLOTS) != hipSuccess) { (void)hipFree(blk); return 3; }
  g_f32k[dev] = blk;
  return 0;
}
static char* f32k_slab(int dev, hipStream_t s) {
  std::lock_guard<std::mutex> lk(g_f32k_mu);
  if (dev < 0 || dev >= 16 || !g_f32k[dev]) return nullptr;
  int pick = -1;
  for (int i = 0; i < F32K_SLOTS; ++i)
    if (g_f32k_used[dev][i] && g_f32k_owner[dev][i] == s) { pick = i; break; }
  if (pick < 0) {
    pick = 0;
    for (int i = 1; i < F32K_SLOTS; ++i)
      if (g_f32k_used[dev][i] < g_f32k_used[dev][pick]) pick = i;
    g_f32k_owner[dev][pick] = s;
  }
  g_f32k_used[dev][pick] = ++g_f32k_clock;
  return g_f32k[dev] + (size_t)pick * F32K_SLAB;
}
bool gemm_f32_ksplit_reserved() {
  int dev = 0;
  if (hipGetDevice(&dev) != hipSuccess || dev < 0 || dev >= 16) return false;
  std::lock_guard<std::mutex> lk(g_f32k_mu);
  return g_f32k[dev] != nullptr;
}

int launch_gemm_f32(const float* A, int lda, const float* W, int ldw, int M, int N, int K,
                    const GemmEpi& e, hipStream_t s, bool allow_ksplit) {
  if (M <= 0 || N <= 0 || K <= 0) return 1;
  if (!e.out_f32 && !e.out_bf16) return 2;
  return gemm_dispatch(GEMM_F32, A, lda, W, ldw, M, N, K, e, s, allow_ksplit);
}

int run_gemm_f32(const float* A, int lda, const float* W, int ldw, int M, int N, int K, const GemmEpi& e, int S, hipStream_t s) {
  const int tiles = ((M + FBM - 1) / FBM) * ((N + FBN - 1) / FBN);
  float* part = nullptr; unsigned* counters = nullptr;
  if (S > 1) {
    int dev = 0;
    (void)hipGetDevice(&dev);
    char* slab = f32k_slab(dev, s);
    if (!slab || tiles > F32K_TILES || (long)tiles * S > F32K_PARTS) return 2;
    counters = reinterpret_cast<unsigned*>(slab); part = reinterpret_cast<float*>(slab + (size_t)F32K_TILES * 4);
  }
  if (vec_ok(A, lda) && vec_ok(W, ldw)) hipLaunchKernelGGL(gemm_f32_kernel<true>, dim3(tiles, S), dim3(256), 0, s, A, lda, W, ldw, M, N, K, e, part, counters);
  else hipLaunchKernelGGL(gemm_f32_kernel<false>, dim3(tiles, S), dim3(256), 0, s, A, lda, W, ldw, M, N, K, e, part, counters);
  return hipGetLastError() == hipSuccess ? 0 : 3;
}

template <bool AKM, bool WKM, bool VEC>
__global__ __launch_bounds__(256) void gemm_f32x_kernel(GemmF32X g) {
  __shared__ __attribute__((aligned(16))) float f32_smem[4 * FBK * FLD];
  const int tid = threadIdx.x;
  const int tiles_m = (g.M + FBM - 1) / FBM;
  const int tn = blockIdx.x / tiles_m, tm = blockIdx.x - tn * tiles_m;
  const int m0 = tm * FBM, n0 = tn * FBN;
  const int zb = blockIdx.y / g.hb, zh = blockIdx.y - zb * g.hb;
  const int nkt = (g.K + FBK - 1) / FBK;
  int kt0 = 0, kt1 = nkt;
  if (g.ksplit > 1) {
    const int per = (nkt + g.ksplit - 1) / g.ksplit;
    kt0 = blockIdx.z * per; kt1 = kt0 + per < nkt ? kt0 + per : nkt;
    if (kt0 >= kt1) return;
  }
  const int kend = kt1 * FBK < g.K ? kt1 * FBK : g.K;
  TileLoad<AKM, VEC> la;
  TileLoad<WKM, VEC> lw;
  la.init(g.A + zb * g.a_sb + zh * g.a_sh, g.lda, g.M, kend, m0, tid);
  lw.init(g.W + zb * g.w_sb + zh * g.w_sh, g.ldw, g.N, kend, n0, tid);
  f32x16 acc;
#pragma unroll
  for (int r = 0; r < 16; ++r) acc[r] = 0.f;
  f32_mainloop(la, lw, kt0, kt1, reinterpret_cast<float (*)[FBK * FLD]>(f32_smem),
               reinterpret_cast<float (*)[FBK * FLD]>(f32_smem + 2 * FBK * FLD), acc);

  float* cz = g.C + zb * g.c_sb + zh * g.c_sh;
  if (g.ksplit > 1) f32x_epi_atomic(g, cz, m0, n0, acc, f32_smem, blockIdx.z == 0);
  else f32x_epi_direct(g, cz, m0, n0, acc);
}

int launch_gemm_f32x(const GemmF32X& g_, hipStream_t s) {
  GemmF32X g = g_;
  if (g.M <= 0 || g.N <= 0 || g.K <= 0 || !g.A || !g.W || !g.C) return 1;
  if (g.batch < 1) g.batch = 1;
  if (g.hb < 1) g.hb = 1;
  if (g.batch % g.hb || g.batch > 65535) return 2;
  if (g.ksplit < 1) g.ksplit = 1;
  if (g.ksplit > 1 && (g.act != ACT_NONE || g.scale || g.resid)) return 2;
  const int nkt = (g.K + FBK - 1) / FBK;
  if (g.ksplit > nkt) g.ksplit = nkt;
  const int tiles = ((g.M + FBM - 1) / FBM) * ((g.N + FBN - 1) / FBN);
  const bool vec = vec_ok(g.A, g.lda, g.a_sb, g.a_sh) && vec_ok(g.W, g.ldw, g.w_sb, g.w_sh);
  const dim3 grid(tiles, g.batch, g.ksplit);
#define F32X_LAUNCH(AK, WK) do { if (vec) hipLaunchKernelGGL((gemm_f32x_kernel<AK, WK, true>), grid, dim3(256), 0, s, g); \
                                 else hipLaunchKernelGGL((gemm_f32x_kernel<AK, WK, false>), grid, dim3(256), 0, s, g); } while (0)
  if (g.a_kmajor && g.w_kmajor) F32X_LAUNCH(true, true);
  else if (g.a_kmajor) F32X_LAUNCH(true, false);
  else if (g.w_kmajor) F32X_LAUNCH(false, true);
  else F32X_LAUNCH(false, false);
#undef F32X_LAUNCH
  return hipGetLastError() == hipSuccess ? 0 : 3;
}
```

### dinov2_od_amd/csrc/gemm_pp.hip

```cpp
#include <mutex>
#include "dod_common.h"
#include "gemm_epi.h"
#include <cstdlib>
#include <cstring>

#define PPM 256
#define PPN 256
#define PPK 64
#define PP_PLANE (256 * 64)
#define PP_TILE (4 * PP_PLANE)

__device__ __forceinline__ int pp_swz(int row, int chunk) { return chunk ^ (((row >> 3) & 1) << 1); }


#ifdef DINODET_TUNING
__device__ unsigned long long* g_pp_stamps = nullptr;
extern "C" int dod_debug_pp_stamps(void* dev_buf) {
  unsigned long long* p = (unsigned long long*)dev_buf;
  return hipMemcpyToSymbol(HIP_SYMBOL(g_pp_stamps), &p, sizeof(p)) == hipSuccess ? 0 : 3;
}
#define PP_STAMPS_DECL unsigned long long* const stamps = g_pp_stamps;
#else
#define PP_STAMPS_DECL unsigned long long* const stamps = nullptr;
#endif
// ... 355 lines not shown
    if (pass) __syncthreads();
#pragma unroll
    for (int ii = 0; ii < 2; ++ii)
#pragma unroll
      for (int j = 0; j < 2; ++j) stage_acc(smem, PITCH, grp_ * 64 + ii * 32 + lr, wq * 64 + j * 32, acc[pass * 2 + ii][j], lg);
    auto rowmap = [&](int row_l) { return m0 + (row_l >> 6) * 128 + pass * 64 + (row_l & 63); };
    stage_row_stats<128, PPN, LN>(smem, PITCH, e, M, tid, rowmap, K, n0);
    __syncthreads();
    if (wide) drain_tile_bf16x8<128, PPN, 512, LN>(smem, PITCH, e, M, N, n0, tid, rowmap);
    else drain_tile<128, PPN, 512, LN>(smem, PITCH, e, cp, M, N, n0, tid, rowmap);
  }
  if (stamps && tid == 0) {
    asm volatile("s_waitcnt vmcnt(0)" ::: "memory");
    unsigned long long* o = stamps + (size_t)blockIdx.x * 8;
    o[0] = ts0; o[1] = ts1; o[2] = ts2; o[3] = __builtin_amdgcn_s_memtime(); o[4] = tr0; o[5] = __builtin_amdgcn_s_memrealtime(); o[6] = blockIdx.x; o[7] = 0;
  }
}


static constexpr int LDSPP = (128 * (PPN * 4 + 16)) > 2 * PP_TILE ? (128 * (PPN * 4 + 16)) : 2 * PP_TILE;

#ifdef DINODET_TUNING
static int wres_grid(int M, int N, int* gm) {
  const int tiles_m = (M + PPM - 1) / PPM, tiles_n = (N + PPN - 1) / PPN;
  const char* v = getenv("DINODET_GEMM_WRES");
  if (v && v[0] == '1' && tiles_n % 2 == 0 && tiles_m >= 32) { *gm = (*gm & ~0x300) | 0x400; return 8 * ((tiles_m + 3) / 4) * (tiles_n / 2); }
  return tiles_m * tiles_n;
}
#else
static int wres_grid(int M, int N, int*) { return ((M + PPM - 1) / PPM) * ((N + PPN - 1) / PPN); }
#endif

static void ppm_attr() {
  static bool done[16] = {};
#define ATTR_(LN_) {reinterpret_cast<const void*>(gemm_ppm_256x256_kernel<false, LN_>), LDSPP}, {reinterpret_cast<const void*>(gemm_ppm_256x256_kernel<true, LN_>), LDSPP},
  static const KernelLds k[] = {ATTR_(LN_NONE) ATTR_(LN_CONS) ATTR_(LN_PROD)};
#undef ATTR_
  gemm_lds_attr_once(done, k, sizeof k / sizeof k[0]);
}

int run_gemm_pp(bool x3, const bf16_t* A, int lda, const bf16_t* W, int ldw, int M, int N, int K, const GemmEpi& e, hipStream_t s) {
  if (K % (x3 ? 32 : PPK) != 0) return 2;
  ppm_attr();
  const int S = e.ksplit > 1 ? e.ksplit : 1;
  int gm = S > 1 ? gemm_tile_mode() & 0xfff : gemm_tile_mode();
  const int tiles = S > 1 ? ((M + PPM - 1) / PPM) * ((N + PPN - 1) / PPN) : wres_grid(M, N, &gm);
#define GO_(LN_) { if (x3) hipLaunchKernelGGL((gemm_ppm_256x256_kernel<true, LN_>), dim3(tiles, S), dim3(512), LDSPP, s, A, lda, W, ldw, M, N, K, e, gm); \
                   else hipLaunchKernelGGL((gemm_ppm_256x256_kernel<false, LN_>), dim3(tiles, S), dim3(512), LDSPP, s, A, lda, W, ldw, M, N, K, e, gm); }
  LN_DISPATCH(e, GO_)
#undef GO_
  return hipGetLastError() == hipSuccess ? 0 : 3;
}

static constexpr int LDSH2 = (128 * (PPN * 4 + 16)) > H2_LDS ? (128 * (PPN * 4 + 16)) : H2_LDS;
int launch_gemm_h2(const void* A, int lda, const void* W, int ldw, int M, int N, int K, const GemmEpi& e, hipStream_t s) {
  if (M <= 0 || N <= 0 || K <= 0) return 1;
  if (K % 32 != 0 || N % 4 != 0 || lda % 16 != 0 || ldw % 16 != 0 || lda < 4 * K || ldw < 3 * K || !e.h2_wexp) return 2;
  if (e.out_f32 && e.ldc % 4 != 0) return 2;
  if (e.resid && e.ldr % 4 != 0) return 2;
  if (!e.out_f32 && !e.out_bf16) return 2;
  { const int No = e.glu ? N / 2 : N;
    if (e.out_h2 && (No % 32 != 0 || e.ldc < 2 * No || e.ldc % 8 != 0 || e.out_split != 0)) return 2;
    if (e.glu && e.out_h2 && (N % 8 != 0)) return 2; }
  return gemm_dispatch(GEMM_H2, A, lda, W, ldw, M, N, K, e, s);
}
int run_gemm_h2(const void* A, int lda, const void* W, int ldw, int M, int N, int K, const GemmEpi& e, hipStream_t s) {
  static bool done[16] = {};
  static const KernelLds k[] = {{reinterpret_cast<const void*>(gemm_h2_256x256_kernel<LN_NONE>), LDSH2}, {reinterpret_cast<const void*>(gemm_h2_256x256_kernel<LN_CONS>), LDSH2},
                                {reinterpret_cast<const void*>(gemm_h2_256x256_kernel<LN_PROD>), LDSH2}};
  gemm_lds_attr_once(done, k, 3);
  const int S = e.ksplit > 1 ? e.ksplit : 1;
  const int gm = S > 1 ? gemm_tile_mode() & 0xfff : gemm_tile_mode();
  const int tiles = ((M + PPM - 1) / PPM) * ((N + PPN - 1) / PPN);
#define GO_(LN_) hipLaunchKernelGGL(gemm_h2_256x256_kernel<LN_>, dim3(tiles, S), dim3(512), LDSH2, s, (const char*)A, lda, (const char*)W, ldw, M, N, K, e, gm);
  LN_DISPATCH(e, GO_)
#undef GO_
  return hipGetLastError() == hipSuccess ? 0 : 3;
}

#define KSR_ROWS 16
template <int LN>
__global__ __launch_bounds__(512) void gemm_ksplit_reduce_kernel(const float* __restrict__ part, long long slice_stride, int S, int R, int N,
                                                                 GemmEpi e, int m_base, int M, int K) {
  __shared__ __attribute__((aligned(16))) char smem[KSR_ROWS * (PPN * 4 + 16)];
  constexpr int PITCH = PPN * 4 + 16;
  const int tid = threadIdx.x;
  const int r0 = blockIdx.x * KSR_ROWS, n0 = blockIdx.y * PPN;
  const int c4 = tid & 63;
#pragma unroll
  for (int rl = tid >> 6; rl < KSR_ROWS; rl += 8) {
    const int r = r0 + rl, n = n0 + 4 * c4;
    float4 acc = make_float4(0.f, 0.f, 0.f, 0.f);
    if (r < R && n < N) {
      const float* p = part + (size_t)r * N + n;
      for (int sl = 0; sl < S; ++sl) {
        const float4 v = *reinterpret_cast<const float4*>(p + (size_t)sl * slice_stride);
        acc.x += v.x; acc.y += v.y; acc.z += v.z; acc.w += v.w;
      }
    }
    *reinterpret_cast<float4*>(smem + rl * PITCH + c4 * 16) = acc;
  }
  auto rowmap = [&](int row_l) { return m_base + r0 + row_l; };
  stage_row_stats<KSR_ROWS, PPN, LN>(smem, PITCH, e, M, tid, rowmap, K, n0);
  __syncthreads();
  const ColParams cp = load_col_params<PPN, LN>(e, n0, N, tid);
  if (drain8_ok(e, N)) drain_tile_bf16x8<KSR_ROWS, PPN, 512, LN>(smem, PITCH, e, M, N, n0, tid, rowmap);
  else drain_tile<KSR_ROWS, PPN, 512, LN>(smem, PITCH, e, cp, M, N, n0, tid, rowmap);
}

#define TAIL_SLOTS 4
#define TAIL_GENS 4
static std::mutex g_tail_mu;
static float* g_tail_scratch[16][TAIL_GENS] = {};
static int g_tail_gen[16] = {};
static size_t g_tail_bytes[16] = {};
static hipStream_t g_tail_owner[16][TAIL_SLOTS] = {};
static unsigned long long g_tail_used[16][TAIL_SLOTS] = {};
static unsigned long long g_tail_clock = 0;
int gemm_tail_reserve(size_t bytes) {
  int dev = 0;
  if (hipGetDevice(&dev) != hipSuccess || dev < 0 || dev >= 16) return 3;
  std::lock_guard<std::mutex> lk(g_tail_mu);
  if (g_tail_bytes[dev] >= bytes) return 0;
  if (g_tail_gen[dev] >= TAIL_GENS) return 3;
  float* blk = nullptr;
  if (hipMalloc((void**)&blk, bytes * TAIL_SLOTS) != hipSuccess) return 3;
  g_tail_scratch[dev][g_tail_gen[dev]++] = blk;
  for (int i = 0; i < TAIL_SLOTS; ++i) { g_tail_used[dev][i] = 0; g_tail_owner[dev][i] = nullptr; }
  g_tail_bytes[dev] = bytes;
  return 0;
}
static float* tail_slab(int dev, hipStream_t s) {
  std::lock_guard<std::mutex> lk(g_tail_mu);
  if (!g_tail_gen[dev]) return nullptr;
  int pick = -1;
  for (int i = 0; i < TAIL_SLOTS; ++i)
    if (g_tail_used[dev][i] && g_tail_owner[dev][i] == s) { pick = i; break; }
  if (pick < 0) {
    pick = 0;
    for (int i = 1; i < TAIL_SLOTS; ++i)
      if (g_tail_used[dev][i] < g_tail_used[dev][pick]) pick = i;
    g_tail_owner[dev][pick] = s;
  }
  g_tail_used[dev][pick] = ++g_tail_clock;
  return (float*)((char*)g_tail_scratch[dev][g_tail_gen[dev] - 1] + (size_t)pick * g_tail_bytes[dev]);
}

size_t gemm_tail_reserved() {
  int dev = 0;
  if (hipGetDevice(&dev) != hipSuccess || dev < 0 || dev >= 16) return 0;
  std::lock_guard<std::mutex> lk(g_tail_mu);
  return g_tail_bytes[dev];
}
float* gemm_tail_slab(hipStream_t s) {
  int dev = 0;
  if (hipGetDevice(&dev) != hipSuccess || dev < 0 || dev >= 16) return nullptr;
  return tail_slab(dev, s);
}

int run_gemm_ksplit_reduce(const float* part, int S, int R, int N, const GemmEpi& e, int m_base, int M, int K, hipStream_t s) {
  const int tiles_n = (N + PPN - 1) / PPN;
#define GO_(LN_) hipLaunchKernelGGL(gemm_ksplit_reduce_kernel<LN_>, dim3((R + KSR_ROWS - 1) / KSR_ROWS, tiles_n), dim3(512), 0, s, part, (long long)R * N, S, R, N, e, m_base, M, K);
  LN_DISPATCH(e, GO_)
#undef GO_
  return hipGetLastError() == hipSuccess ? 0 : 3;
}
```

### dinov2_od_amd/engine.py

```python
import ctypes as C
import os

import torch

from . import _native as nat
from .config import BackboneConfig, DecoderConfig


def default_precision():
    return os.environ.get("DINODET_PRECISION", "bf16x3")


TRAIN_PRECISIONS = ("fp32", "bf16x3")


def check_train_precision(value):
    if value not in TRAIN_PRECISIONS:
        raise ValueError(f"train_precision must be 'fp32' or 'bf16x3', got {value!r}")
    return value


def make_config(bb: BackboneConfig, dc: DecoderConfig, precision: str) -> nat.DodConfig:
    if precision not in nat.PREC:
        raise ValueError(f"precision must be one of {sorted(nat.PREC)}, got {precision!r}")
    c = nat.DodConfig()
    c.hidden, c.layers, c.heads, c.swiglu = bb.hidden, bb.layers, bb.heads, int(bb.swiglu)
    c.patch, c.pos_grid, c.ffn_hidden, c.ln_eps = bb.patch, bb.pos_grid, bb.ffn_hidden, bb.ln_eps
    c.lora_r, c.lora_alpha, c.target_dim = bb.lora_r, bb.lora_alpha, bb.target_dim
    c.num_queries, c.dec_hidden, c.dec_heads, c.dec_layers = dc.num_queries, dc.hidden_dim, dc.nheads, dc.num_layers
    c.num_classes, c.dim_feedforward, c.n_points = dc.num_classes, dc.dim_feedforward, dc.n_points
    c.use_deformable, c.dec_ln_eps = int(dc.use_deformable), dc.ln_eps
    c.precision = nat.PREC[precision]
    return c


class Engine:
    def __init__(self, bb: BackboneConfig, dc: DecoderConfig, precision: str):
        self.bb, self.dc, self.precision = bb, dc, precision
        self._lib = nat.lib()
        self._h = C.c_void_p()
        cfg = make_config(bb, dc, precision)
        nat.check(self._lib.dod_create(C.byref(cfg), C.byref(self._h)))
        self._sig = None
        self._ws = None
        self._device = None
        self._keep = []
        self._tap_bufs = {}
        self.use_graph = os.environ.get("DINODET_HIPGRAPH", "0") == "1"
        self._graphs = {}
        self.micro_streams = max(1, int(os.environ.get("DINODET_MICRO_STREAMS", "2")))
        self.micro_min_rows = int(os.environ.get("DINODET_MICRO_MIN_ROWS", "10000"))
        self.micro_min_batch = int(os.environ.get("DINODET_MICRO_MIN_BATCH", "2"))
        self._micro = {}

    def close(self):
        if self._h:
            self._lib.dod_destroy(self._h)
            self._h = C.c_void_p()

    def __del__(self):
        try:
            self.close()
        except Exception:
            pass

    @staticmethod
    def signature(named):
        return tuple((k, t.data_ptr(), t._version, tuple(t.shape)) for k, t in named)

    def sync_weights(self, named):
        sig = self.signature(named)
        if sig == self._sig:
            return
        self._keep = []
        devs = {t.device for _, t in named}
        if len(devs) != 1:
            raise RuntimeError(f"parameters live on several devices ({sorted(map(str, devs))}): one replica per GPU")
        dev = next(iter(devs))
        if dev.type != "cuda":
            raise RuntimeError(f"parameters are on {dev}: the MI355X path has no CPU fallback")
        with torch.cuda.device(dev):
            for k, t in named:
                if t.dtype == torch.bfloat16 and t.is_contiguous():
                    dt = nat.DOD_BF16
                else:
                    dt = nat.DOD_F32
                    if t.dtype != torch.float32 or not t.is_contiguous():
                        t = t.detach().to(torch.float32).contiguous()
                        self._keep.append(t)
                shape = (C.c_int64 * max(t.dim(), 1))(*t.shape)
                nat.check(self._lib.dod_set_weight(self._h, k.encode(), nat.ptr(t), shape, t.dim(), dt), self._h)
            nat.check(self._lib.dod_finalize_weights(self._h, nat.stream_ptr()), self._h)
        self._keep = []
        self._sig = sig
        self._device = dev
        self._ws = None
        self._micro = {}
        self._graphs = {}

    def _workspace(self, nbytes, device):
        if self._ws is None or self._ws.numel() < nbytes or self._ws.device != device:
            self._ws = torch.empty(nbytes, dtype=torch.uint8, device=device)
        return self._ws

    def _on_device(self, x):
        if self._device is not None and x.device != self._device:
            raise RuntimeError(f"input is on {x.device} but the model's parameters are on {self._device}")
        return torch.cuda.device(x.device)

    @staticmethod
    def _check_pixels(x):
        if x.dim() != 4:
            raise ValueError(f"pixel_values must be [batch, 3, H, W], got shape {tuple(x.shape)}")
        if x.shape[1] != 3:
            raise ValueError("Make sure that the channel dimension of the pixel values match with the one set in "
                             f"the configuration. Expected 3 but got {x.shape[1]}.")
        if not x.is_cuda:
            raise RuntimeError("pixel_values must be on the GPU: the MI355X path has no CPU fallback")
        return x.detach().to(torch.float32).contiguous()

    def _forward_graph(self, x):
        key = (tuple(x.shape), x.device)
        ent = self._graphs.get(key)
        if ent is None:
            xs = x.clone()
            B, _, H, W = x.shape
            K = self.micro_streams if (self._micro_ok(B, H, W) and B % self.micro_streams == 0) else 1
            Bk = B // K
            parts = [(xs[k * Bk:(k + 1) * Bk], torch.empty(self._lib.dod_workspace_bytes(self._h, Bk, H, W), dtype=torch.uint8, device=x.device))
                     for k in range(K)]
            out = torch.empty(B, self.dc.num_queries, self.dc.num_classes + 4, dtype=torch.float32, device=x.device)
            for k, (xk, wk) in enumerate(parts):
                self._launch_forward(xk, wk, out[k * Bk:(k + 1) * Bk])
            torch.cuda.synchronize(x.device)
            side = [torch.cuda.Stream(device=x.device) for _ in range(K - 1)]
            g = torch.cuda.CUDAGraph()
            with torch.cuda.graph(g, capture_error_mode="thread_local"):
                cur = torch.cuda.current_stream(x.device)
                for st in side:
                    st.wait_stream(cur)
                self._launch_forward(parts[0][0], parts[0][1], out[:Bk])
                for k, st in enumerate(side, start=1):
                    with torch.cuda.stream(st):
                        self._launch_forward(parts[k][0], parts[k][1], out[k * Bk:(k + 1) * Bk])
                for st in side:
                    cur.wait_stream(st)
            ent = (g, xs, out, [w for _, w in parts], side)
            self._graphs[key] = ent
        g, xs, out = ent[0], ent[1], ent[2]
        xs.copy_(x)
        g.replay()
        return out

    def _launch_forward(self, x, ws=None, det=None):
        B, _, H, W = x.shape
        nbytes = self._lib.dod_workspace_bytes(self._h, B, H, W)
        if nbytes == 0:
            raise ValueError(f"unsupported input {tuple(x.shape)}")
        if ws is None:
            ws = self._workspace(nbytes, x.device)
        if det is None:
            det = torch.empty(B, self.dc.num_queries, self.dc.num_classes + 4, dtype=torch.float32, device=x.device)
        nat.check(self._lib.dod_forward(self._h, nat.ptr(x), B, H, W, nat.ptr(det), nat.ptr(ws), ws.numel(),
                                        nat.stream_ptr()), self._h)
        return det

    def _micro_ok(self, B, H, W):
        K = self.micro_streams
        return (K >= 2 and B >= max(self.micro_min_batch, K)
                and B * self._lib.dod_num_tokens(self._h, H, W) >= self.micro_min_rows)

    def _launch_micro(self, x):
        B, _, H, W = x.shape
        K = self.micro_streams
        if not self._micro_ok(B, H, W) or self._tap_bufs:
            return self._launch_forward(x)
        sizes = [B // K + (1 if k < B % K else 0) for k in range(K)]
        offs = [sum(sizes[:k]) for k in range(K)]
        key = (tuple(sizes), H, W, x.device)
        st = self._micro.get(key)
        if st is None:
            wss = []
            for bk in sizes:
                nb = self._lib.dod_workspace_bytes(self._h, bk, H, W)
                if nb == 0:
                    raise ValueError(f"unsupported input {tuple(x.shape)}")
                wss.append(torch.empty(nb, dtype=torch.uint8, device=x.device))
            st = (wss, [torch.cuda.Stream(device=x.device) for _ in range(K - 1)])
            self._micro[key] = st
        wss, side = st
        det = torch.empty(B, self.dc.num_queries, self.dc.num_classes + 4, dtype=torch.float32, device=x.device)
        cur = torch.cuda.current_stream(x.device)
        nat.check(self._lib.dod_prepare(self._h, H, W, nat.stream_ptr()), self._h)
        for sd in side:
            sd.wait_stream(cur)
        self._launch_forward(x[:sizes[0]], wss[0], det[:sizes[0]])
        for k, sd in enumerate(side, start=1):
            with torch.cuda.stream(sd):
                self._launch_forward(x[offs[k]:offs[k] + sizes[k]], wss[k], det[offs[k]:offs[k] + sizes[k]])
        for sd in side:
            cur.wait_stream(sd)
        return det

    def forward(self, pixel_values, named):
        x = self._check_pixels(pixel_values)
        self.sync_weights(named)
        with self._on_device(x):
            if self.use_graph and not torch.cuda.is_current_stream_capturing() and not self._tap_bufs:
                return self._forward_graph(x)
            return self._launch_micro(x)

    def forward_u8(self, pixels_hwc, named):
        x = pixels_hwc
        if x.dim() != 4 or x.shape[-1] != 3 or x.dtype != torch.uint8:
            raise ValueError(f"expected uint8 [batch, H, W, 3], got {x.dtype} {tuple(x.shape)}")
        if not x.is_cuda:
            raise RuntimeError("pixels must be on the GPU: the MI355X path has no CPU fallback")
        x = x.contiguous()
        self.sync_weights(named)
        B, H, W, _ = x.shape
        nbytes = self._lib.dod_workspace_bytes(self._h, B, H, W)
        if nbytes == 0:
            raise ValueError(f"unsupported input {tuple(x.shape)}")
        with self._on_device(x):
            ws = self._workspace(nbytes, x.device)
            det = torch.empty(B, self.dc.num_queries, self.dc.num_classes + 4, dtype=torch.float32, device=x.device)
            nat.check(self._lib.dod_forward_u8(self._h, nat.ptr(x), B, H, W, nat.ptr(det), nat.ptr(ws), ws.numel(), nat.stream_ptr()), self._h)
        return det

    def backbone_forward(self, pixel_values, named):
        x = self._check_pixels(pixel_values)
        self.sync_weights(named)
        B, _, H, W = x.shape
        nbytes = self._lib.dod_workspace_bytes(self._h, B, H, W)
        if nbytes == 0:
            raise ValueError(f"unsupported input {tuple(x.shape)}")
        with self._on_device(x):
            ws = self._workspace(nbytes, x.device)
            N = self._lib.dod_num_tokens(self._h, H, W)
            feats = torch.empty(B, N, self.bb.out_dim, dtype=torch.float32, device=x.device)
            nat.check(self._lib.dod_backbone_forward(self._h, nat.ptr(x), B, H, W, nat.ptr(feats), nat.ptr(ws),
                                                     ws.numel(), nat.stream_ptr()), self._h)
        return feats

    def backbone_prefix(self, pixel_values, named, nblocks):
        x = self._check_pixels(pixel_values)
        self.sync_weights(named)
        B, _, H, W = x.shape
        nbytes = self._lib.dod_workspace_bytes(self._h, B, H, W)
        if nbytes == 0:
            raise ValueError(f"unsupported input {tuple(x.shape)}")
        with self._on_device(x):
            ws = self._workspace(nbytes, x.device)
            N = self._lib.dod_num_tokens(self._h, H, W)
            out = torch.empty(B, N, self.bb.hidden, dtype=torch.float32, device=x.device)
            nat.check(self._lib.dod_backbone_prefix(self._h, nat.ptr(x), B, H, W, int(nblocks), nat.ptr(out), nat.ptr(ws), ws.numel(),
                                                    nat.stream_ptr()), self._h)
        return out

    def decoder_forward(self, memory, named):
        if memory.dim() != 3 or memory.shape[-1] != self.dc.hidden_dim:
            raise ValueError(f"src must be [batch, seq_len, {self.dc.hidden_dim}], got {tuple(memory.shape)}")
        if not memory.is_cuda:
            raise RuntimeError("src must be on the GPU: the MI355X path has no CPU fallback")
        m = memory.detach().to(torch.float32).contiguous()
        self.sync_weights(named)
        B, N, _ = m.shape
        nbytes = self._lib.dod_decoder_workspace_bytes(self._h, B, N)
        with self._on_device(m):
            ws = self._workspace(nbytes, m.device)
            det = torch.empty(B, self.dc.num_queries, self.dc.num_classes + 4, dtype=torch.float32, device=m.device)
            nat.check(self._lib.dod_decoder_forward(self._h, nat.ptr(m), B, N, nat.ptr(det), nat.ptr(ws), ws.numel(),
                                                    nat.stream_ptr()), self._h)
        return det

    PROFILE_CLASSES = {"gemm_bf16": 0, "attn_bf16": 1, "gemm_f32": 2, "attn_f32": 3, "layernorm": 4, "gemm_fp8": 6}

    def profile(self, enable):
        nat.check(self._lib.dod_profile(self._h, int(bool(enable))), self._h)

    def profile_read(self):
        out = {}
        for name, cls in self.PROFILE_CLASSES.items():
            ms, fl, n = C.c_double(), C.c_double(), C.c_int()
            nat.check(self._lib.dod_profile_read(self._h, cls, C.byref(ms), C.byref(fl), C.byref(n)), self._h)
            out[name] = {"ms": ms.value, "flops": fl.value, "launches": n.value}
        return out

    def set_tap(self, stage, shape, device):
        buf = torch.zeros(*shape, dtype=torch.float32, device=device)
        self._tap_bufs[stage] = buf
        nat.check(self._lib.dod_set_tap(self._h, stage, nat.ptr(buf)), self._h)
        return buf

    def clear_taps(self):
        for st in list(self._tap_bufs):
            nat.check(self._lib.dod_set_tap(self._h, st, C.c_void_p(0)), self._h)
        self._tap_bufs = {}


def split_detections(det, num_classes):
    return {"pred_logits": det[..., :num_classes], "pred_boxes": det[..., num_classes:]}
```

### include/dinodet.h

```cpp
#ifndef DINODET_H
#define DINODET_H
#include <stddef.h>
#include <stdint.h>

#ifdef __cplusplus
extern "C" {
#endif

typedef struct dod_handle dod_handle;

enum dod_dtype { DOD_F32 = 0, DOD_BF16 = 1 };

enum dod_status {
  DOD_OK = 0,
  DOD_ERR_INVALID = 1,
  DOD_ERR_MISSING = 2,
  DOD_ERR_STATE = 3,
  DOD_ERR_HIP = 4
};

enum dod_precision {
  DOD_PREC_FP32 = 0,
  DOD_PREC_BF16 = 1,
  DOD_PREC_BF16X3 = 3,
  DOD_PREC_FP8 = 2,
  DOD_PREC_FP16X2 = 4
};

typedef struct dod_config {
  int32_t hidden;
  int32_t layers;
  int32_t heads;
  int32_t swiglu;
  int32_t patch;
  int32_t pos_grid;
  int32_t ffn_hidden;
  float   ln_eps;
  int32_t lora_r;
  float   lora_alpha;
  int32_t target_dim;
  int32_t num_queries;
  int32_t dec_hidden;
  int32_t dec_heads;
  int32_t dec_layers;
  int32_t num_classes;
  int32_t dim_feedforward;
  int32_t n_points;
  int32_t use_deformable;
  float   dec_ln_eps;
  int32_t precision;
} dod_config;

int dod_create(const dod_config* cfg, dod_handle** out);
void dod_destroy(dod_handle* h);
const char* dod_last_error(const dod_handle* h);

int dod_set_weight(dod_handle* h, const char* key, const void* dev_ptr, const int64_t* shape, int ndim, int dtype );

int dod_finalize_weights(dod_handle* h, void* stream);

int dod_prepare(dod_handle* h, int H, int W, void* stream);

size_t dod_workspace_bytes(const dod_handle* h, int B, int H, int W);
int dod_num_tokens(const dod_handle* h, int H, int W);

int dod_forward(dod_handle* h, const float* pixels, int B, int H, int W, float* detections,
                void* workspace, size_t workspace_bytes, void* stream);

int dod_forward_u8(dod_handle* h, const uint8_t* pixels_hwc, int B, int H, int W, float* detections,
                   void* workspace, size_t workspace_bytes, void* stream);

int dod_backbone_forward(dod_handle* h, const float* pixels, int B, int H, int W, float* features,
                         void* workspace, size_t workspace_bytes, void* stream);
int dod_backbone_prefix(dod_handle* h, const float* pixels, int B, int H, int W, int nblocks, float* x_out,
                        void* workspace, size_t workspace_bytes, void* stream);

int dod_decoder_forward(dod_handle* h, const float* memory, int B, int N, float* detections,
                        void* workspace, size_t workspace_bytes, void* stream);
size_t dod_decoder_workspace_bytes(const dod_handle* h, int B, int N);

int dod_set_tap(dod_handle* h, int stage, float* dst);

int dod_profile(dod_handle* h, int enable);
int dod_profile_read(dod_handle* h, int cls, double* ms, double* flops, int* launches);

enum dod_act { DOD_ACT_NONE = 0, DOD_ACT_RELU = 1, DOD_ACT_GELU = 2, DOD_ACT_SIGMOID = 3,
               DOD_ACT_SWIGLU_PAIRS = 4 };

int dod_op_linear(int in_dtype, const void* A, int lda, const void* W, int ldw, int M, int N, int K,
                  const float* bias, const float* scale, const float* resid, int ldr,
                  void* out, int out_dtype, int ldc, int act, void* stream);
int dod_op_gemm_f32x(const float* A, int lda, int a_kmajor, long long a_sb, long long a_sh,
                     const float* W, int ldw, int w_kmajor, long long w_sb, long long w_sh,
                     float* C, int ldc, long long c_sb, long long c_sh,
                     int M, int N, int K, int batch, int hb, float alpha, int accumulate, int ksplit, void* stream);
int dod_op_gemm_f32x3(const float* A, int lda, int a_kmajor, long long a_sb, long long a_sh,
                      const float* W, int ldw, int w_kmajor, long long w_sb, long long w_sh,
                      float* C, int ldc, long long c_sb, long long c_sh,
                      int M, int N, int K, int batch, int hb, float alpha, int accumulate, int ksplit, void* stream);
int dod_op_linear_f32x3(const float* X, int ldx, const float* W, const float* bias, const float* scale, const float* resid, int ldr,
                        int M, int N, int K, float* Y, int ldy, int act, void* stream);
int dod_op_linear_fp8(const void* A, int lda, const float* a_scale, const void* W, int ldw, const float* w_scale,
                      int M, int N, int K, const float* bias, const float* scale, const float* resid, int ldr,
                      void* out, int out_dtype, int ldc, int act, void* stream);
int dod_op_quant_rows_fp8(const void* x, int in_dtype, int ld, int rows, int cols, void* q, int ldq, float* scale,
                          void* stream);
int dod_op_quant_mx_fp8(const void* x, int in_dtype, int ld, int rows, int cols, void* q, int ldq, void* block_scales, void* stream);
int dod_op_linear_fp8_mx(const void* A, int lda, const void* a_block_scales, const void* W, int ldw, const float* w_scale,
                         int M, int N, int K, const float* bias, const float* scale, const float* resid, int ldr,
                         void* out, int out_dtype, int ldc, int act, void* stream);
int dod_op_linear_fp8_glu_mx(const void* A, int lda, const float* a_scale, const void* W, int ldw, const float* w_scale,
                             int M, int N, int K, const float* bias, void* out_q, int ldq, void* out_block_scales, void* stream);
int dod_op_linear_fp8_mx2(const void* A, int lda, const void* a_block_scales, const void* W, int ldw, const void* w_block_scales,
                          int M, int N, int K, const float* bias, const float* scale, const float* resid, int ldr,
                          void* out, int out_dtype, int ldc, int act, void* glu_out_block_scales, void* stream);
int dod_op_split_pair(const float* x, int ld, int rows, int cols, void* out, void* stream);
int dod_op_linear_x3(const void* A2, const void* W2, int M, int N, int K, const float* bias, const float* scale,
                     const float* resid, int ldr, void* out, int out_layout, int ldc, int act, void* stream);
int dod_op_attention_x3(const void* qkv2, void* ctx2, int B, int N, int heads, float scale, void* stream);
int dod_op_attention_x3_h2(const void* qkv2, void* ctx_h2, int B, int N, int heads, float scale, void* stream);
int dod_op_split_h2(const float* x, int ld, int rows, int cols, void* out, void* wexp, void* stream);
int dod_op_linear_h2(const void* A, const void* W, const void* wexp, int M, int N, int K, const float* bias, const float* scale,
                     const float* resid, int ldr, void* out, int out_layout, int ldc, int act, void* stream);
typedef struct dod_ln_fold {
  const void* stats;
  const float* csum;
  void* op_out;
  void* part;
  const void* shift;
  const void* part_in;
  void* stats_out;
  float eps;
} dod_ln_fold;
int dod_op_linear_ln(int family, const void* A, const void* W, const void* wexp, int M, int N, int K, const float* bias, const float* scale,
                     const float* resid, int ldr, void* out, int out_layout, int ldc, int act, const dod_ln_fold* ln, void* stream);
int dod_op_rowstats(const float* x, int rows, int D, float eps, void* op_out, int family, void* stats, void* stream);
int dod_op_ln_finalize(const void* part, int rows, int D, float eps, void* stats, void* stream);
int dod_op_layernorm(const float* x, const float* add, const float* gamma, const float* beta, float eps,
                     int rows, int D, void* out, int out_dtype, void* stream);
int dod_op_attention_bf16(const void* qkv, void* ctx, int B, int N, int heads, float scale, void* stream);
int dod_op_attention_bf16_mx(const void* qkv, void* ctx_q8, void* ctx_bs, int B, int N, int heads, float scale, void* stream);
int dod_op_attention_f32(const float* q, const float* k, const float* v, float* o, int ldq, int ldk, int ldv,
                         int ldo, int Lq, int Lk, int B, int heads, int dh, float scale, void* stream);
int dod_op_deform_sample(const float* proj, int ldp, const float* values, int B, int Q, int N, int Hd, int P,
                         int dh, int h, int w, float* out, void* stream);
int dod_op_pos_resize(const float* pos_in, int G, int gh, int gw, int D, float* pos_out, void* stream);
int dod_op_im2col(const float* img, int B, int H, int W, int patch, int Kp, void* out, int out_dtype, void* stream);

typedef struct dod_detection {
  int64_t image_id;
  int32_t category_id;
  int32_t query;
  float bbox[4];
  float score;
  int32_t reserved;
} dod_detection;
size_t dod_postprocess_workspace_bytes(int B, int Q, int C);
int dod_postprocess(const float* det, int B, int Q, int C, const int64_t* image_ids, float threshold,
                    dod_detection* out, int64_t max_out, int64_t* count, void* workspace, size_t workspace_bytes,
                    void* stream);

size_t dod_detect_workspace_bytes(int B, int Q, int C, int K);
int dod_detect(const float* det, int B, int Q, int C, int first_class, const float* sizes, float threshold, int K,
               float iou_threshold, int class_agnostic, int clamp, float* scores, int32_t* labels, int32_t* queries, float* boxes,
               int32_t* counts, void* workspace, size_t workspace_bytes, void* stream);

size_t dod_detect_views_workspace_bytes(int V, int Q, int C, int K);
int dod_detect_views(const float* det, int B, int V, int Q, int C, const int32_t* view_offsets, const int32_t* view_rects,
                     const uint8_t* view_flips, const float* sizes, int first_class, float threshold, int K, float iou_threshold,
                     int nms_metric, int class_agnostic, int clamp, float edge_margin, float* scores, int32_t* labels, int32_t* views,
                     int32_t* queries, float* boxes, int32_t* counts, void* workspace, size_t workspace_bytes, void* stream);

size_t dod_fuse_views_workspace_bytes(int V, int Q, int C, int K);
int dod_fuse_views(const float* det, int B, int V, int Q, int C, const int32_t* view_offsets, const int32_t* view_rects,
                   const uint8_t* view_flips, const float* sizes, int first_class, float threshold, int K, float iou_threshold,
                   int class_agnostic, int clamp, float edge_margin, int conf, float* scores, int32_t* labels, int32_t* views,
                   int32_t* queries, float* boxes, int32_t* members, int32_t* counts, void* workspace, size_t workspace_bytes,
                   void* stream);

typedef struct dod_draw_layer {
  const float* boxes;
  const int32_t* counts;
  const int32_t* labels;
  const float* scores;
  int32_t K;
  int32_t format;
  float score_threshold;
  int32_t use_palette;
  uint8_t color[4];
} dod_draw_layer;
typedef struct dod_draw_style {
  int32_t thickness;
  int32_t fill_alpha;
  int32_t font_scale;
  int32_t palette_size;
  const uint8_t* palette;
  const uint8_t* names;
  int32_t n_names;
  int32_t name_len;
  const uint8_t* font;
} dod_draw_style;
int dod_draw_detections(const void* images, int images_fp32, int B, int H, int W, const dod_draw_layer* below,
                        const dod_draw_layer* above, const dod_draw_style* style, uint8_t* out, void* stream);

int dod_preprocess(const uint8_t* src, const int64_t* src_offs, const int32_t* heights, const int32_t* widths, int B,
                   int max_h, int max_w, int out_h, int out_w, uint8_t* tmp, const int64_t* tmp_offs, float* out,
                   void* stream);

int dod_preprocess_u8(const uint8_t* src, const int64_t* src_offs, const int32_t* heights, const int32_t* widths, int B,
                      int max_h, int max_w, int out_h, int out_w, uint8_t* tmp, const int64_t* tmp_offs, uint8_t* out_hwc,
                      void* stream);

int dod_preprocess_aug(const uint8_t* src, const int64_t* src_offs, const int32_t* heights, const int32_t* widths, int B,
                       const int32_t* crops, const uint8_t* flips, const float* jitter, uint64_t* lsum, int max_crop_h,
                       int max_crop_w, int out_h, int out_w, uint8_t* tmp, const int64_t* tmp_offs, float* out, void* stream);

int dod_preprocess_aug_u8(const uint8_t* src, const int64_t* src_offs, const int32_t* heights, const int32_t* widths, int B,
                          const int32_t* crops, const uint8_t* flips, const float* jitter, uint64_t* lsum, int max_crop_h,
                          int max_crop_w, int out_h, int out_w, uint8_t* tmp, const int64_t* tmp_offs, uint8_t* out_hwc,
                          void* stream);
// ... 177 lines not shown
```

Baseline: 2605 images/s.

## Run backbone micro-batches on side streams and join into one batched decoder

Adds a native split forward that runs the backbone on K micro-batches in concurrent streams. Each stream also projects its memory rows (value or KV projections) into shared buffers. After the join, a single decoder runs over the whole batch, replacing K small per-stream decoders whose launches and small GEMMs were poorly utilised. This applies when B*queries fits under a row cap. The cost is serialising the decoder tail after the join, a larger KV workspace (per layer), and stream/event management inside the library.

```diff
diff --git a/dinov2_od_amd/_native.py b/dinov2_od_amd/_native.py
--- a/dinov2_od_amd/_native.py
+++ b/dinov2_od_amd/_native.py
@@ -103,6 +103,10 @@
     "dod_workspace_bytes": (_SZ, [_P, _I, _I, _I]),
     "dod_num_tokens": (_I, [_P, _I, _I]),
     "dod_forward": (_I, [_P, _P, _I, _I, _I, _P, _P, _SZ, _P]),
+    "dod_forward_split": (_I, [_P, _P, _I, _I, _I, _P, _P, _SZ, _P, _I]),
+    "dod_workspace_bytes_split": (_SZ, [_P, _I, _I, _I, _I]),
+    "dod_max_micro_batches": (_I, []),
+    "dod_joint_decoder_max_rows": (_I, []),
     "dod_forward_u8": (_I, [_P, _P, _I, _I, _I, _P, _P, _SZ, _P]),
     "dod_backbone_forward": (_I, [_P, _P, _I, _I, _I, _P, _P, _SZ, _P]),
     "dod_backbone_prefix": (_I, [_P, _P, _I, _I, _I, _I, _P, _P, _SZ, _P]),
diff --git a/dinov2_od_amd/csrc/dod_api.hip b/dinov2_od_amd/csrc/dod_api.hip
--- a/dinov2_od_amd/csrc/dod_api.hip
+++ b/dinov2_od_amd/csrc/dod_api.hip
@@ -35,10 +35,10 @@
   return true;
 }
 
-static std::atomic<int> g_options[DOD_OPT_COUNT] = {{-1}, {-1}, {-1}, {-1}, {-1}, {-1}, {-1}, {-1}, {-1}, {-1}, {-1}};
+static std::atomic<int> g_options[DOD_OPT_COUNT] = {{-1}, {-1}, {-1}, {-1}, {-1}, {-1}, {-1}, {-1}, {-1}, {-1}, {-1}, {-1}};
 int dod_option(int which) { return which >= 0 && which < DOD_OPT_COUNT ? g_options[which].load() : -1; }
 static const char* const k_option_names[DOD_OPT_COUNT] = {"tailsplit", "dec_fused_split", "mha_chunk_images", "no_fused_patch", "ln_fold", "deterministic", "f32_ksplit",
-                                                       "attn_bwd_flash", "epi_regmath", "f32x3_tile", "attn_diet"};
+                                                       "attn_bwd_flash", "epi_regmath", "f32x3_tile", "attn_diet", "joint_decoder"};
 
 static std::atomic<long> g_form_launches[FORM_COUNT];
 static const char* const k_form_names[FORM_COUNT] = {"bf16_128_r2", "bf16_128_r3", "bf16_m16", "k64", "ppm", "x3_16w", "x3_pp", "h2", "fp8_rows", "fp8mx_256x128",
@@ -59,6 +59,7 @@
   if (name && !strcmp(name, "f32_ksplits")) return gemm_f32_ksplit_count();
   if (name && !strcmp(name, "epi_regmath")) return gemm_epi_regmath_count();
   if (name && !strcmp(name, "attn_diet")) return attn_half_tile_count();
+  if (name && !strcmp(name, "joint_decoders")) return joint_decoder_count();
   if (name && !strcmp(name, "f32x3_launches")) return gemm_f32x3_count(0);
   if (name && !strcmp(name, "f32x3_wide_launches")) return gemm_f32x3_count(1);
   if (name && !strcmp(name, "optim_launches")) return optim_launch_count();
@@ -120,6 +121,9 @@
   if (!h) return;
   for (auto& r : h->prof) { (void)hipEventDestroy(r.a); (void)hipEventDestroy(r.b); }
   for (auto e : h->evpool) (void)hipEventDestroy(e);
+  for (auto e : h->side_done) (void)hipEventDestroy(e);
+  if (h->fork_ev) (void)hipEventDestroy(h->fork_ev);
+  for (auto s : h->side) (void)hipStreamDestroy(s);
   for (void* p : h->owned) (void)hipFree(p);
   delete h;
 }
@@ -218,6 +222,32 @@
   return decoder_impl(h, bw.mem, B, N, dw, det, (hipStream_t)stream);
 }
 
+int dod_max_micro_batches(void) { return max_micro_batches(); }
+int dod_joint_decoder_max_rows(void) { return joint_decoder_max_rows(); }
+
+size_t dod_workspace_bytes_split(const dod_handle* h, int B, int H, int W, int n_micro) {
+  if (n_micro == 1) return dod_workspace_bytes(h, B, H, W);
+  if (!h || B <= 0 || H < h->cfg.patch || W < h->cfg.patch || n_micro < 1 || n_micro > B || n_micro > max_micro_batches()) return 0;
+  const int N = dod_num_tokens(h, H, W);
+  Carver cj(nullptr), cs(nullptr);
+  carve_split(h, cj, B, N, n_micro, true, nullptr, nullptr);
+  carve_split(h, cs, B, N, n_micro, false, nullptr, nullptr);
+  return (cj.off > cs.off ? cj.off : cs.off) + 256;
+}
+
+int dod_forward_split(dod_handle* h, const float* pixels, int B, int H, int W, float* det, void* workspace, size_t wsb, void* stream, int n_micro) {
+  int rc;
+  if (!check_common(h, B, H, W, &rc)) return rc;
+  if (n_micro < 1 || n_micro > max_micro_batches()) return fail(h, DOD_ERR_INVALID, "n_micro %d outside 1..%d (one GEMM scratch slab per concurrently launching stream)", n_micro, max_micro_batches());
+  if (n_micro > B) return fail(h, DOD_ERR_INVALID, "n_micro %d exceeds the batch of %d", n_micro, B);
+  if (n_micro == 1) return dod_forward(h, pixels, B, H, W, det, workspace, wsb, stream);
+  if (!pixels || !det || !workspace) return fail(h, DOD_ERR_INVALID, "null buffer");
+  if (!h->taps.empty()) return fail(h, DOD_ERR_STATE, "debug taps are set: they follow the single-stream forward (dod_forward)");
+  const size_t need = dod_workspace_bytes_split(h, B, H, W, n_micro);
+  if (wsb < need) return fail(h, DOD_ERR_STATE, "workspace too small: %zu < %zu", wsb, need);
+  return forward_split_impl(h, pixels, B, H, W, det, workspace, wsb, (hipStream_t)stream, n_micro);
+}
+
 int dod_forward_u8(dod_handle* h, const uint8_t* pixels_hwc, int B, int H, int W, float* det, void* workspace, size_t wsb, void* stream) {
   int rc;
   if (!check_common(h, B, H, W, &rc)) return rc;
diff --git a/dinov2_od_amd/csrc/dod_common.h b/dinov2_od_amd/csrc/dod_common.h
--- a/dinov2_od_amd/csrc/dod_common.h
+++ b/dinov2_od_amd/csrc/dod_common.h
@@ -24,6 +24,7 @@
        DOD_OPT_EPI_REGMATH,
        DOD_OPT_F32X3_TILE,
        DOD_OPT_ATTN_DIET,
+       DOD_OPT_JOINT_DECODER,
        DOD_OPT_COUNT };
 int dod_option(int which);
 long gemm_tail_split_count();
@@ -276,6 +277,8 @@
 size_t gemm_tail_reserved();
 float* gemm_tail_slab(hipStream_t s);
 bool gemm_f32_ksplit_reserved();
+int gemm_tail_slots();
+int gemm_f32_ksplit_slots();
 int launch_bcast_rows(const float* src, float* dst, int B, int rows, int D, hipStream_t s);
 
 int launch_deform_sample(const float* proj, int ldp, const float* values, int B, int Q, int N, int Hd, int P, int dh,
diff --git a/dinov2_od_amd/csrc/dod_forward.hip b/dinov2_od_amd/csrc/dod_forward.hip
--- a/dinov2_od_amd/csrc/dod_forward.hip
+++ b/dinov2_od_amd/csrc/dod_forward.hip
@@ -1,11 +1,12 @@
 #include "dod_internal.h"
 
+#include <atomic>
 #include <cmath>
 #include <cstdlib>
 
 using namespace dod;
 
-size_t dod::carve_decoder(const dod_handle* h, Carver& c, int B, int N, DecWS* w, bool need_mem_op) {
+size_t dod::carve_decoder(const dod_handle* h, Carver& c, int B, int N, DecWS* w, bool need_mem_op, int kv_layers) {
   const dod_config& g = h->cfg;
   const size_t BQ = (size_t)B * g.num_queries, Dd = g.dec_hidden, M = (size_t)B * N;
   DecWS t;
@@ -25,7 +26,8 @@
     if (!h->finalized) uniq = g.dec_layers;
     t.values = (float*)c.take(M * Dd * 4 * (size_t)(uniq > 0 ? uniq : 1)); t.kv = nullptr;
   } else {
-    t.values = nullptr; t.kv = (float*)c.take(M * 2 * Dd * 4);
+    t.values = nullptr; t.kv = (float*)c.take(M * 2 * Dd * 4 * (size_t)(kv_layers > 1 ? kv_layers : 1));
+    if (kv_layers > 1) t.kv_stride = M * 2 * Dd;
   }
   if (w) *w = t;
   return c.off;
@@ -322,7 +324,37 @@
   return DOD_OK;
 }
 
-int dod::decoder_impl(dod_handle* h, const void* mem_op, int B, int N, const DecWS& ws, float* det, hipStream_t s, bool l0_only) {
+int dod::decoder_memory_impl(dod_handle* h, const void* mem_op, int Mtot, int r0, int rows, const DecWS& ws, hipStream_t s) {
+  const dod_config& g = h->cfg;
+  const bool bf = is_bf16(h), x3 = is_x3(h) && ws.mem2;
+  const int Dd = g.dec_hidden;
+  const void* op = (const char*)mem_op + (size_t)r0 * Dd * (bf ? 2 : 4);
+  bf16_t* mem2 = x3 ? ws.mem2 + (size_t)r0 * 2 * Dd : nullptr;
+  if (x3) KCHK(h, launch_split2((const float*)op, Dd, mem2, rows, Dd, s));
+  if (!g.use_deformable) return DOD_OK;
+  int u = 0;
+  for (int j = 0; j < g.dec_layers; ++j) {
+    const DLayer& L = h->DL[j];
+    if (L.vp_alias >= 0) continue;
+    float* dst = ws.values + ((size_t)u * Mtot + r0) * Dd; ++u;
+    int rc;
+    if (x3 && L.vp_w2) rc = linear3(h, mem2, L.vp_w2, rows, Dd, Dd, epi(L.vp_b, dst, nullptr, Dd), s);
+    else rc = linear(h, bf, op, Dd, L.vp_w, Dd, rows, Dd, Dd, epi(L.vp_b, dst, nullptr, Dd), s);
+    if (rc) return rc;
+  }
+  return DOD_OK;
+}
+
+int dod::decoder_kv_impl(dod_handle* h, const void* mem_op, int Mtot, int r0, int rows, int layer, const DecWS& ws, hipStream_t s) {
+  const bool bf = is_bf16(h), x3 = is_x3(h) && ws.mem2;
+  const int Dd = h->cfg.dec_hidden;
+  const DLayer& L = h->DL[layer];
+  float* dst = ws.kv + (size_t)layer * ws.kv_stride + (size_t)r0 * 2 * Dd;
+  if (x3 && L.ca_kv_w2) return linear3(h, ws.mem2 + (size_t)r0 * 2 * Dd, L.ca_kv_w2, rows, 2 * Dd, Dd, epi(L.ca_kv_b, dst, nullptr, 2 * Dd), s);
+  return linear(h, bf, (const char*)mem_op + (size_t)r0 * Dd * (bf ? 2 : 4), Dd, L.ca_kv_w, Dd, rows, 2 * Dd, Dd, epi(L.ca_kv_b, dst, nullptr, 2 * Dd), s);
+}
+
+int dod::decoder_impl(dod_handle* h, const void* mem_op, int B, int N, const DecWS& ws, float* det, hipStream_t s, bool l0_only, bool mem_done) {
   const dod_config& g = h->cfg;
   const bool bf = is_bf16(h);
   const int Dd = g.dec_hidden, Q = g.num_queries, Hd = g.dec_heads, Pn = g.n_points, Fd = g.dim_feedforward, C = g.num_classes;
@@ -333,21 +365,12 @@
   int rc;
   if (!l0_only) tap(h, 1000, mem_op, bf, (size_t)M * Dd, s);
   const bool x3 = is_x3(h) && ws.mem2;
-  if (x3 && !l0_only) KCHK(h, launch_split2((const float*)mem_op, Dd, ws.mem2, M, Dd, s));
   const bool l0_const = !l0_only && h->l0_tgt && (!g.use_deformable || h->l0_proj);
   if (!l0_const) KCHK(h, launch_bcast_rows(h->query, ws.tgt, 1, Q, Dd, s));
   int fh = 0, fw = 0;
+  if (!l0_only && !mem_done) { rc = decoder_memory_impl(h, mem_op, M, 0, M, ws, s); if (rc) return rc; }
   if (g.use_deformable && !l0_only) {
     spatial_factor(N, &fh, &fw);
-    int u = 0;
-    for (int j = 0; j < g.dec_layers; ++j) {
-      DLayer& L = h->DL[j];
-      if (L.vp_alias >= 0) continue;
-      float* dst = ws.values + (size_t)u * M * Dd; ++u;
-      if (x3 && L.vp_w2) rc = linear3(h, ws.mem2, L.vp_w2, M, Dd, Dd, epi(L.vp_b, dst, nullptr, Dd), s);
-      else rc = linear(h, bf, mem_op, Dd, L.vp_w, Dd, M, Dd, Dd, epi(L.vp_b, dst, nullptr, Dd), s);
-      if (rc) return rc;
-    }
     tap(h, 2000, ws.values, false, (size_t)M * Dd, s);
   }
   const float sscale = 1.0f / std::sqrt((float)dh);
@@ -419,10 +442,9 @@
       if (shared0 && !const0) KCHK(h, launch_bcast_rows(ws.tgt, ws.tgt + (size_t)Q * Dd, B - 1, Q, Dd, s));
       rc = qlinear(ws.tgt, Dd, L.ca_q_w, L.ca_q_w3, BQ, Dd, epi(L.ca_q_b, ws.qd, nullptr, Dd), tgt3); if (rc) return rc;
       tgt3 = nullptr;
-      if (x3 && L.ca_kv_w2) rc = linear3(h, ws.mem2, L.ca_kv_w2, M, 2 * Dd, Dd, epi(L.ca_kv_b, ws.kv, nullptr, 2 * Dd), s);
-      else rc = linear(h, bf, mem_op, Dd, L.ca_kv_w, Dd, M, 2 * Dd, Dd, epi(L.ca_kv_b, ws.kv, nullptr, 2 * Dd), s);
-      if (rc) return rc;
-      AttnF32 a; a.q = ws.qd; a.k = ws.kv; a.v = ws.kv + Dd; a.o = ws.att; a.ldq = Dd; a.ldk = a.ldv = 2 * Dd; a.ldo = Dd;
+      if (!mem_done) { rc = decoder_kv_impl(h, mem_op, M, 0, M, j, ws, s); if (rc) return rc; }
+      const float* kv = ws.kv + (size_t)j * ws.kv_stride;
+      AttnF32 a; a.q = ws.qd; a.k = kv; a.v = kv + Dd; a.o = ws.att; a.ldq = Dd; a.ldk = a.ldv = 2 * Dd; a.ldo = Dd;
       a.Lq = Q; a.Lk = N; a.B = B; a.heads = Hd; a.dh = dh; a.scale = sscale;
       const bool o3 = fuse3 && splits(L.ca_out_w3, BQ, Dd, Dd, ACT_NONE);
       if (o3) a.o3 = ws.a3;
@@ -439,3 +461,77 @@
   rc = linear(h, false, ws.hb, Dd / 2, h->bb2_w, Dd / 2, BQ, 4, Dd / 2, epi(h->bb2_b, det + C, nullptr, C + 4, ACT_SIGMOID), s); if (rc) return rc;
   return DOD_OK;
 }
+
+int dod::max_micro_batches() { const int a = gemm_tail_slots(), b = gemm_f32_ksplit_slots(); return a < b ? a : b; }
+
+size_t dod::carve_split(const dod_handle* h, Carver& c, int B, int N, int K, bool joint, BbWS* bw, DecWS* dw) {
+  for (int k = 0; k < K; ++k) {
+    const int Bk = B / K + (k < B % K ? 1 : 0);
+    carve_backbone(h, c, Bk, N, bw ? bw + k : nullptr);
+    if (!joint) carve_decoder(h, c, Bk, N, dw ? dw + k : nullptr, false);
+  }
+  if (joint) carve_decoder(h, c, B, N, dw, true, h->cfg.use_deformable ? 1 : h->cfg.dec_layers);
+  return c.off;
+}
+
+#define JOINT_DECODER_MAX_ROWS 3200
+static std::atomic<long> g_joint_decoders;
+long dod::joint_decoder_count() { return g_joint_decoders.load(); }
+int dod::joint_decoder_max_rows() { return JOINT_DECODER_MAX_ROWS; }
+
+namespace {
+int split_streams(dod_handle* h, int K) {
+  if (!h->fork_ev) HIPCHK(h, hipEventCreateWithFlags(&h->fork_ev, hipEventDisableTiming));
+  while ((int)h->side.size() < K - 1) {
+    hipStream_t st = nullptr; hipEvent_t ev = nullptr;
+    HIPCHK(h, hipStreamCreateWithFlags(&st, hipStreamNonBlocking));
+    const hipError_t e = hipEventCreateWithFlags(&ev, hipEventDisableTiming);
+    if (e != hipSuccess) { (void)hipStreamDestroy(st); return fail(h, DOD_ERR_HIP, "hipEventCreateWithFlags: %s", hipGetErrorString(e)); }
+    h->side.push_back(st); h->side_done.push_back(ev);
+  }
+  return DOD_OK;
+}
+}
+
+int dod::forward_split_impl(dod_handle* h, const float* pixels, int B, int H, int W, float* det, void* workspace, size_t wsb, hipStream_t s, int K) {
+  const dod_config& g = h->cfg;
+  const int N = (H / g.patch) * (W / g.patch) + 1, Dd = g.dec_hidden;
+  const size_t img = (size_t)3 * H * W, det_img = (size_t)g.num_queries * (g.num_classes + 4);
+  const int opt = dod_option(DOD_OPT_JOINT_DECODER);
+  const bool joint = opt >= 0 ? opt != 0 : (long)B * g.num_queries <= JOINT_DECODER_MAX_ROWS;
+  if (joint) ++g_joint_decoders;
+  std::vector<BbWS> bw(K);
+  std::vector<DecWS> dw(joint ? 1 : K);
+  Carver c(align_ws(workspace));
+  carve_split(h, c, B, N, K, joint, bw.data(), dw.data());
+  CARVE_FITS(h, c, workspace, wsb)
+  int rc = split_streams(h, K); if (rc) return rc;
+  rc = prepare_impl(h, H, W, s); if (rc) return rc;
+  HIPCHK(h, hipEventRecord(h->fork_ev, s));
+  int forked = 0;
+  for (; forked < K - 1 && !rc; ++forked) {
+    const hipError_t e = hipStreamWaitEvent(h->side[forked], h->fork_ev, 0);
+    if (e != hipSuccess) { rc = fail(h, DOD_ERR_HIP, "hipStreamWaitEvent (fork): %s", hipGetErrorString(e)); break; }
+  }
+  const size_t op_row = (size_t)Dd * (is_bf16(h) ? 2 : 4);
+  int b0 = 0;
+  for (int k = 0; k < K && !rc; ++k) {
+    const int Bk = B / K + (k < B % K ? 1 : 0);
+    hipStream_t sk = k == 0 ? s : h->side[k - 1];
+    if (joint) bw[k].mem = (char*)dw[0].mem_op + (size_t)b0 * N * op_row;
+    rc = backbone_impl(h, pixels + (size_t)b0 * img, Bk, H, W, bw[k], nullptr, true, sk);
+    if (!rc && !joint) rc = decoder_impl(h, bw[k].mem, Bk, N, dw[k], det + (size_t)b0 * det_img, sk);
+    if (!rc && joint) {
+      rc = decoder_memory_impl(h, dw[0].mem_op, B * N, b0 * N, Bk * N, dw[0], sk);
+      for (int j = 0; j < g.dec_layers && !rc && !g.use_deformable; ++j) rc = decoder_kv_impl(h, dw[0].mem_op, B * N, b0 * N, Bk * N, j, dw[0], sk);
+    }
+    b0 += Bk;
+  }
+  for (int i = 0; i < forked; ++i) {
+    hipError_t e = hipEventRecord(h->side_done[i], h->side[i]);
+    if (e == hipSuccess) e = hipStreamWaitEvent(s, h->side_done[i], 0);
+    if (e != hipSuccess && !rc) rc = fail(h, DOD_ERR_HIP, "join of micro-batch %d: %s", i + 1, hipGetErrorString(e));
+  }
+  if (!rc && joint) rc = decoder_impl(h, dw[0].mem_op, B, N, dw[0], det, s, false, true);
+  return rc;
+}
diff --git a/dinov2_od_amd/csrc/dod_internal.h b/dinov2_od_amd/csrc/dod_internal.h
--- a/dinov2_od_amd/csrc/dod_internal.h
+++ b/dinov2_od_amd/csrc/dod_internal.h
@@ -62,6 +62,9 @@
   struct ProfRec { hipEvent_t a, b; int cls; double flops; };
   std::vector<ProfRec> prof;
   std::vector<hipEvent_t> evpool;
+  std::vector<hipStream_t> side;
+  std::vector<hipEvent_t> side_done;
+  hipEvent_t fork_ev = nullptr;
 };
 
 namespace dod {
@@ -117,9 +120,10 @@
 #define CARVE_FITS(h, c, workspace, wsb)                                                                                      \
   if ((size_t)((c).base - (char*)(workspace)) + (c).off > (wsb))                                                              \
     return dod::fail(h, DOD_ERR_STATE, "internal: workspace carve %zu exceeds the %zu bytes provided", (size_t)((c).base - (char*)(workspace)) + (c).off, (size_t)(wsb));
-struct DecWS { float *tgt, *t2, *att, *samp, *qkv, *proj, *ffn, *hb, *qd; void* mem_op; float* values; float* kv; bf16_t* a3; bf16_t* a3b; bf16_t* mem2; };
+struct DecWS { float *tgt, *t2, *att, *samp, *qkv, *proj, *ffn, *hb, *qd; void* mem_op; float* values; float* kv; bf16_t* a3; bf16_t* a3b; bf16_t* mem2;
+               size_t kv_stride = 0; };
 struct BbWS { float* x; void *y, *qkv, *ctx, *hbuf, *gated, *mem; float* rs; unsigned char* bs; unsigned char* bsx; float2 *lnp, *lns, *lns2; };
-size_t carve_decoder(const dod_handle* h, Carver& c, int B, int N, DecWS* w, bool need_mem_op);
+size_t carve_decoder(const dod_handle* h, Carver& c, int B, int N, DecWS* w, bool need_mem_op, int kv_layers = 1);
 size_t carve_backbone(const dod_handle* h, Carver& c, int B, int N, BbWS* w);
 
 int finalize_impl(dod_handle* h, hipStream_t s);
@@ -127,6 +131,14 @@
 int prepare_impl(dod_handle* h, int H, int W, hipStream_t s);
 int backbone_impl(dod_handle* h, const float* pixels, int B, int H, int W, const BbWS& ws, float* feat_f32, bool want_mem, hipStream_t s,
                   int stop_blocks = -1, float* x_out = nullptr, const unsigned char* pixels_u8 = nullptr);
-int decoder_impl(dod_handle* h, const void* mem_op, int B, int N, const DecWS& ws, float* det, hipStream_t s, bool l0_only = false);
+int decoder_impl(dod_handle* h, const void* mem_op, int B, int N, const DecWS& ws, float* det, hipStream_t s, bool l0_only = false, bool mem_done = false);
+int decoder_memory_impl(dod_handle* h, const void* mem_op, int Mtot, int r0, int rows, const DecWS& ws, hipStream_t s);
+int decoder_kv_impl(dod_handle* h, const void* mem_op, int Mtot, int r0, int rows, int layer, const DecWS& ws, hipStream_t s);
+
+long joint_decoder_count();
+int joint_decoder_max_rows();
+int max_micro_batches();
+size_t carve_split(const dod_handle* h, Carver& c, int B, int N, int K, bool joint, BbWS* bw, DecWS* dw);
+int forward_split_impl(dod_handle* h, const float* pixels, int B, int H, int W, float* det, void* workspace, size_t wsb, hipStream_t s, int K);
 
 }
diff --git a/dinov2_od_amd/csrc/gemm_f32.hip b/dinov2_od_amd/csrc/gemm_f32.hip
--- a/dinov2_od_amd/csrc/gemm_f32.hip
+++ b/dinov2_od_amd/csrc/gemm_f32.hip
@@ -210,6 +210,7 @@
   g_f32k_used[dev][pick] = ++g_f32k_clock;
   return g_f32k[dev] + (size_t)pick * F32K_SLAB;
 }
+int gemm_f32_ksplit_slots() { return F32K_SLOTS; }
 bool gemm_f32_ksplit_reserved() {
   int dev = 0;
   if (hipGetDevice(&dev) != hipSuccess || dev < 0 || dev >= 16) return false;
diff --git a/dinov2_od_amd/csrc/gemm_pp.hip b/dinov2_od_amd/csrc/gemm_pp.hip
--- a/dinov2_od_amd/csrc/gemm_pp.hip
+++ b/dinov2_od_amd/csrc/gemm_pp.hip
@@ -531,6 +531,7 @@
   std::lock_guard<std::mutex> lk(g_tail_mu);
   return g_tail_bytes[dev];
 }
+int gemm_tail_slots() { return TAIL_SLOTS; }
 float* gemm_tail_slab(hipStream_t s) {
   int dev = 0;
   if (hipGetDevice(&dev) != hipSuccess || dev < 0 || dev >= 16) return nullptr;
diff --git a/dinov2_od_amd/engine.py b/dinov2_od_amd/engine.py
--- a/dinov2_od_amd/engine.py
+++ b/dinov2_od_amd/engine.py
@@ -48,7 +48,7 @@
         self._tap_bufs = {}
         self.use_graph = os.environ.get("DINODET_HIPGRAPH", "0") == "1"
         self._graphs = {}
-        self.micro_streams = max(1, int(os.environ.get("DINODET_MICRO_STREAMS", "2")))
+        self.micro_streams = min(max(1, int(os.environ.get("DINODET_MICRO_STREAMS", "2"))), self._lib.dod_max_micro_batches())
         self.micro_min_rows = int(os.environ.get("DINODET_MICRO_MIN_ROWS", "10000"))
         self.micro_min_batch = int(os.environ.get("DINODET_MICRO_MIN_BATCH", "2"))
         self._micro = {}
@@ -125,27 +125,20 @@
         if ent is None:
             xs = x.clone()
             B, _, H, W = x.shape
-            K = self.micro_streams if (self._micro_ok(B, H, W) and B % self.micro_streams == 0) else 1
-            Bk = B // K
-            parts = [(xs[k * Bk:(k + 1) * Bk], torch.empty(self._lib.dod_workspace_bytes(self._h, Bk, H, W), dtype=torch.uint8, device=x.device))
-                     for k in range(K)]
+            K = self.micro_streams if self._micro_ok(B, H, W) else 1
             out = torch.empty(B, self.dc.num_queries, self.dc.num_classes + 4, dtype=torch.float32, device=x.device)
-            for k, (xk, wk) in enumerate(parts):
-                self._launch_forward(xk, wk, out[k * Bk:(k + 1) * Bk])
+            if K == 1 or self._joint(B):
+                keep = torch.empty(self._split_bytes(B, H, W, K), dtype=torch.uint8, device=x.device)
+                launch = lambda: self._launch_split(xs, keep, out, K)
+            else:
+                keep = self._fork_state(B, H, W, K, x.device)
+                launch = lambda: self._launch_fork(xs, out, keep)
+            launch()
             torch.cuda.synchronize(x.device)
-            side = [torch.cuda.Stream(device=x.device) for _ in range(K - 1)]
             g = torch.cuda.CUDAGraph()
             with torch.cuda.graph(g, capture_error_mode="thread_local"):
-                cur = torch.cuda.current_stream(x.device)
-                for st in side:
-                    st.wait_stream(cur)
-                self._launch_forward(parts[0][0], parts[0][1], out[:Bk])
-                for k, st in enumerate(side, start=1):
-                    with torch.cuda.stream(st):
-                        self._launch_forward(parts[k][0], parts[k][1], out[k * Bk:(k + 1) * Bk])
-                for st in side:
-                    cur.wait_stream(st)
-            ent = (g, xs, out, [w for _, w in parts], side)
+                launch()
+            ent = (g, xs, out, keep)
             self._graphs[key] = ent
         g, xs, out = ent[0], ent[1], ent[2]
         xs.copy_(x)
@@ -170,26 +163,35 @@
         return (K >= 2 and B >= max(self.micro_min_batch, K)
                 and B * self._lib.dod_num_tokens(self._h, H, W) >= self.micro_min_rows)
 
-    def _launch_micro(self, x):
-        B, _, H, W = x.shape
-        K = self.micro_streams
-        if not self._micro_ok(B, H, W) or self._tap_bufs:
-            return self._launch_forward(x)
+    def _split_bytes(self, B, H, W, K):
+        nbytes = self._lib.dod_workspace_bytes_split(self._h, B, H, W, K)
+        if nbytes == 0:
+            raise ValueError(f"unsupported input {(B, 3, H, W)} as {K} micro-batches")
+        return nbytes
+
+    def _launch_split(self, x, ws, det, K):
+        B, _, H, W = x.shape
+        nat.check(self._lib.dod_forward_split(self._h, nat.ptr(x), B, H, W, nat.ptr(det), nat.ptr(ws), ws.numel(), nat.stream_ptr(), K),
+                  self._h)
+        return det
+
+    def _joint(self, B):
+        return B * self.dc.num_queries <= self._lib.dod_joint_decoder_max_rows()
+
+    def _fork_state(self, B, H, W, K, device):
         sizes = [B // K + (1 if k < B % K else 0) for k in range(K)]
-        offs = [sum(sizes[:k]) for k in range(K)]
-        key = (tuple(sizes), H, W, x.device)
-        st = self._micro.get(key)
-        if st is None:
-            wss = []
-            for bk in sizes:
-                nb = self._lib.dod_workspace_bytes(self._h, bk, H, W)
-                if nb == 0:
-                    raise ValueError(f"unsupported input {tuple(x.shape)}")
-                wss.append(torch.empty(nb, dtype=torch.uint8, device=x.device))
-            st = (wss, [torch.cuda.Stream(device=x.device) for _ in range(K - 1)])
-            self._micro[key] = st
-        wss, side = st
-        det = torch.empty(B, self.dc.num_queries, self.dc.num_classes + 4, dtype=torch.float32, device=x.device)
+        wss = []
+        for bk in sizes:
+            nb = self._lib.dod_workspace_bytes(self._h, bk, H, W)
+            if nb == 0:
+                raise ValueError(f"unsupported input {(B, 3, H, W)}")
+            wss.append(torch.empty(nb, dtype=torch.uint8, device=device))
+        return sizes, wss, [torch.cuda.Stream(device=device) for _ in range(K - 1)]
+
+    def _launch_fork(self, x, det, st):
+        sizes, wss, side = st
+        H, W = x.shape[2:]
+        offs = [sum(sizes[:k]) for k in range(len(sizes))]
         cur = torch.cuda.current_stream(x.device)
         nat.check(self._lib.dod_prepare(self._h, H, W, nat.stream_ptr()), self._h)
         for sd in side:
@@ -202,6 +204,22 @@
             cur.wait_stream(sd)
         return det
 
+    def _launch_micro(self, x):
+        B, _, H, W = x.shape
+        K = self.micro_streams
+        if not self._micro_ok(B, H, W) or self._tap_bufs:
+            return self._launch_forward(x)
+        key = (B, K, H, W, x.device)
+        st = self._micro.get(key)
+        det = torch.empty(B, self.dc.num_queries, self.dc.num_classes + 4, dtype=torch.float32, device=x.device)
+        if self._joint(B):
+            if st is None:
+                st = self._micro[key] = torch.empty(self._split_bytes(B, H, W, K), dtype=torch.uint8, device=x.device)
+            return self._launch_split(x, st, det, K)
+        if st is None:
+            st = self._micro[key] = self._fork_state(B, H, W, K, x.device)
+        return self._launch_fork(x, det, st)
+
     def forward(self, pixel_values, named):
         x = self._check_pixels(pixel_values)
         self.sync_weights(named)
diff --git a/include/dinodet.h b/include/dinodet.h
--- a/include/dinodet.h
+++ b/include/dinodet.h
@@ -66,6 +66,12 @@
 
 int dod_forward(dod_handle* h, const float* pixels, int B, int H, int W, float* detections,
                 void* workspace, size_t workspace_bytes, void* stream);
+
+size_t dod_workspace_bytes_split(const dod_handle* h, int B, int H, int W, int n_micro);
+int dod_max_micro_batches(void);
+int dod_joint_decoder_max_rows(void);
+int dod_forward_split(dod_handle* h, const float* pixels, int B, int H, int W, float* detections,
+                      void* workspace, size_t workspace_bytes, void* stream, int n_micro);
 
 int dod_forward_u8(dod_handle* h, const uint8_t* pixels_hwc, int B, int H, int W, float* detections,
                    void* workspace, size_t workspace_bytes, void* stream);
```

After: 2609 images/s (median of 2 runs). No clear change (+0.1%).
